# AtomGradient/swift-qwen3-tts

Measured on AMD Instinct MI355X. Metric: codec_tokens_per_s, higher is better.
Workload: dtype bf16

## Files before the change

### include/q3tts.h

```cpp
#ifndef Q3TTS_H
#define Q3TTS_H

#include <stddef.h>
#include <stdint.h>

#ifdef __cplusplus
extern "C" {
#endif

#define Q3TTS_ABI_VERSION 4

typedef struct q3tts_model q3tts_model;

typedef enum {
    Q3TTS_OK = 0,
    Q3TTS_ERR_MODEL_NOT_INITIALIZED = 1,
    Q3TTS_ERR_GENERATION_FAILED = 2,
    Q3TTS_ERR_INVALID_INPUT = 3,
    Q3TTS_ERR_AUDIO_DECODING_FAILED = 4,
    Q3TTS_ERR_AUDIO_ENCODING_FAILED = 5,
    Q3TTS_ERR_IO = 6,
    Q3TTS_ERR_DEVICE = 7,
    Q3TTS_ERR_CANCELLED = 8,
    Q3TTS_ERR_BUSY = 9
// ... 327 lines not shown
    float* rider_ss_out;
} q3tts_gemm_debug;
q3tts_status q3tts_debug_gemm(q3tts_model* m, q3tts_gemm_debug* a);

typedef struct {
    int32_t kind, geometry_only, split;
    int32_t B, Tmax, ppf, hist, margin;
    int32_t Cin, N, K, dil;
    int32_t ldx, ldo, ldr, ldx2;
    int32_t act, pre_act, shift, reflect, post_C;
    int32_t x_f32, res_is_out;
    int32_t family;
    int32_t BN;
    int32_t pro, pw_depth, KT, X32, CT2, PT, wdb;
    int32_t grid_x, grid_y, grid_z;
    int64_t lds_bytes;
    const int32_t* frames;
    const void* x;
    const float* x2;
    const float* w;
    const float* w2;
    const float* bias;
    const float* bias2;
    const float* scale;
    const float* snake_alpha;
    const float* snake_beta;
    const float* act2_alpha;
    const float* act2_beta;
    const float* post_alpha;
    const float* post_beta;
    const void* res;
    void* out;
    void* out2;
    float* pcm;
    int32_t* nonfinite;
} q3tts_conv_debug;
q3tts_status q3tts_debug_conv(q3tts_model* m, q3tts_conv_debug* a);

typedef struct {
    int32_t op, check_only;
    int32_t p[16];
    float f[4];
    const void* in[8];
    int64_t in_bytes[8];
    void* io[4];
    int64_t io_bytes[4];
} q3tts_rowop_debug;
q3tts_status q3tts_debug_rowop(q3tts_model* m, q3tts_rowop_debug* a);

typedef struct {
    float temperature;
    int32_t top_k;
    float top_p;
    float rep_penalty;
    uint64_t seed;
    uint32_t row0;
    int32_t mask_eos;
} q3tts_lm_sampling_params;
typedef struct {
    int32_t slot, n_trailing, max_frames;
    uint32_t row_key;
    int32_t text_open;
    int32_t pad_;
    q3tts_lm_sampling_params sp;
} q3tts_lm_admit_desc;
typedef struct {
    int32_t slot, src_row, n_new, close, max_frames, pad_;
} q3tts_lm_text_desc;
typedef struct {
    int32_t op, check_only;
    int32_t p[32];
    const void* in[14];
    int64_t in_bytes[14];
    void* io[18];
    int64_t io_bytes[18];
} q3tts_lmop_debug;
q3tts_status q3tts_debug_lmop(q3tts_model* m, q3tts_lmop_debug* a);

q3tts_status q3tts_debug_codec_stage(q3tts_model* m, const int32_t* codes, int32_t n_frames,
                                     const char* stage, float* out, int64_t cap_floats, int32_t* T, int32_t* C);

q3tts_status q3tts_debug_prefix_states(q3tts_model* m, int32_t* n_states, int64_t* device_bytes, int64_t* n_restored);

q3tts_status q3tts_debug_stretch_rows(q3tts_model* m, const float* x, const int32_t* lens, const int32_t* hops, int32_t B,
                                      int64_t x_stride, float* y, int64_t y_stride);

q3tts_status q3tts_debug_resample_ratio(q3tts_model* m, const float* x, const int32_t* lens, int32_t B, int64_t row_stride, int64_t in_units,
                                        int64_t out_units, int32_t centred, int32_t clamp, int32_t hist, float* y, int64_t y_stride);

q3tts_status q3tts_debug_codec_stream_slots(q3tts_model* m, const int32_t* codes, const int32_t* n_frames, int32_t n_reqs,
                                            int32_t max_frames, int32_t slots, int32_t burst, int32_t chunk_frames, int32_t window,
                                            int32_t lookahead, float* pcm);

q3tts_status q3tts_debug_build_decode_codes(q3tts_model* m, const int32_t* refs, const int32_t* ref_T, const int32_t* gen,
                                            const int32_t* n_frames, int32_t R, int32_t gen_stride, int32_t Fdec, int32_t misalign,
                                            int32_t* out);

void q3tts_debug_set_codec_scratch(uint64_t bytes);

void q3tts_debug_reload_env(void);

q3tts_status q3tts_debug_frontend_stage(q3tts_model* m, const float* audio, int64_t n_samples, const char* stage,
                                        float* out, int64_t cap_floats, int32_t* T, int32_t* C);

#ifdef __cplusplus
}
#endif
#endif
```

### swift-qwen3-tts_amd/csrc/api.cc

```cpp
#include <atomic>
#include <cmath>
#include <cstdio>
#include <cstring>
#include <thread>
#include <vector>

#include "codec.h"
#include "comm.h"
#include "engine.h"
#include "tokenizer.h"

using q3::EngineGroup;

struct q3tts_session {
    q3tts_model* m = nullptr;
};

struct q3tts_model {
    std::unique_ptr<EngineGroup> eng;
    std::unique_ptr<q3tts_session> session;
    std::atomic<std::thread::id> owner{std::thread::id()};
    std::atomic<int> depth{0};
};
struct q3tts_tokenizer {
// ... 556 lines not shown
    return guarded(m, [&] {
        Q3_CHECK(m && audio && out, 3, "Invalid input: null argument");
        Q3_CHECK(sample_rate == 24000, 3,
                 "Invalid input: Only 24kHz audio is supported for speaker embedding extraction");
        m->eng->lane0().speaker_embedding(audio, n_samples, out, cap);
        m->eng->timing = m->eng->lane0().timing;
    });
}

q3tts_status q3tts_debug_frontend_stage(q3tts_model* m, const float* audio, int64_t n_samples, const char* stage, float* out,
                                        int64_t cap_floats, int32_t* T, int32_t* C) {
    return guarded(m, [&] {
        Q3_CHECK(m && audio && stage && out && T && C, 3, "Invalid input: null argument");
        m->eng->lane0().debug_frontend_stage(audio, n_samples, stage, out, cap_floats, T, C);
    });
}

q3tts_status q3tts_tokenizer_load(const char* path, q3tts_tokenizer** out) {
    return guarded(nullptr, [&] {
        Q3_CHECK(path && out, 3, "Invalid input: null argument");
        auto t = std::make_unique<q3tts_tokenizer>();
        const std::string p = path;
        if (p.size() > 5 && p.compare(p.size() - 5, 5, ".json") == 0) t->tok.load_json_file(p);
        else t->tok.load(p);
        *out = t.release();
    });
}
void q3tts_tokenizer_free(q3tts_tokenizer* t) { delete t; }
q3tts_status q3tts_tokenizer_encode(const q3tts_tokenizer* t, const char* utf8, int32_t* ids, int32_t cap, int32_t* n) {
    return guarded(nullptr, [&] {
        Q3_CHECK(t && utf8 && n, 3, "Invalid input: null argument");
        const std::vector<int32_t> v = t->tok.encode(utf8);
        *n = int32_t(v.size());
        Q3_CHECK(ids == nullptr || cap >= *n, 3, "Invalid input: output buffer too small for the token ids");
        if (ids) std::memcpy(ids, v.data(), v.size() * 4);
    });
}

q3tts_status q3tts_last_timing(const q3tts_model* m, q3tts_timing* out) {
    if (!m || !out) return Q3TTS_ERR_INVALID_INPUT;
    *out = m->eng->timing;
    return Q3TTS_OK;
}

q3tts_status q3tts_debug_prepare_inputs(q3tts_model* m, const q3tts_request* req, uint16_t* input_embeds,
                                        int32_t cap_prompt, int32_t* n_prompt, uint16_t* trailing, int32_t cap_trailing,
                                        int32_t* n_trailing, uint16_t* tts_pad) {
    return guarded(m, [&] {
        Q3_CHECK(m && req && input_embeds && n_prompt && trailing && n_trailing && tts_pad, 3, "Invalid input: null argument");
        m->eng->lane0().debug_prepare_inputs(*req, input_embeds, cap_prompt, n_prompt, trailing, cap_trailing, n_trailing, tts_pad);
    });
}

q3tts_status q3tts_debug_generate_forced(q3tts_model* m, const q3tts_request* reqs, int32_t n_reqs,
                                         const q3tts_sampling* sampling, const int32_t* forced_codes, int32_t n_frames,
                                         uint16_t* talker_logits, uint16_t* cp_logits, int32_t* sampled) {
    return guarded(m, [&] {
        Q3_CHECK(m && reqs && n_frames > 0, 3, "Invalid input: null argument");
        q3tts_sampling sp;
        if (sampling) sp = *sampling;
        else q3tts_default_sampling(&sp);
        q3::DebugOpts d;
        d.forced_codes = forced_codes;
        d.frames = n_frames;
        d.talker_logits = talker_logits;
        d.cp_logits = cp_logits;
        d.sampled = sampled;
        std::vector<q3tts_result> res((size_t)(n_reqs));
        m->eng->generate(reqs, n_reqs, sp, nullptr, nullptr, res.data(), &d);
        q3tts_result_free(res.data(), n_reqs);
    });
}

q3tts_status q3tts_debug_sample(q3tts_model* m, const uint16_t* logits, int32_t rows, int32_t V,
                                const q3tts_sampling* sampling, const uint8_t* seen, int32_t suppress_lo,
                                int32_t suppress_hi, int32_t eos_id, uint32_t row0, uint32_t draw, int32_t* tokens) {
    return guarded(m, [&] {
        Q3_CHECK(m && logits && sampling && tokens, 3, "Invalid input: null argument");
        q3::check_row_sampling(*sampling, rows);
        m->eng->lane0().debug_sample(logits, rows, V, *sampling, seen, suppress_lo, suppress_hi, eos_id, row0, draw, tokens);
    });
}

q3tts_status q3tts_debug_text_resume(q3tts_model* m, int32_t H, int32_t V, const uint16_t* tables, const int32_t* codes,
                                     const uint16_t* text_row, uint16_t* out_h, float* out_ss, int32_t* out_state) {
    return guarded(m, [&] {
        Q3_CHECK(m, 3, "Invalid input: null argument");
        m->eng->lane0().debug_text_resume(H, V, tables, codes, text_row, out_h, out_ss, out_state);
    });
}

q3tts_status q3tts_debug_linear(q3tts_model* m, const uint16_t* x, const uint16_t* W, const uint16_t* bias, int32_t M,
                                int32_t K, int32_t N, uint16_t* y) {
    return guarded(m, [&] {
        Q3_CHECK(m && x && W && y, 3, "Invalid input: null argument");
        m->eng->lane0().debug_linear(x, W, bias, M, K, N, y);
    });
}

q3tts_status q3tts_debug_attention(q3tts_model* m, const q3tts_attn_debug* a) {
    return guarded(m, [&] {
        Q3_CHECK(m && a, 3, "Invalid input: null argument");
        m->eng->lane0().debug_attention(*a);
    });
}

q3tts_status q3tts_debug_gemm(q3tts_model* m, q3tts_gemm_debug* a) {
    if (a && a->geometry_only) {
        return guarded(nullptr, [&] {
            q3::GemmArgs ga{};
            q3::NormRowsArgs na{};
            q3::Engine::debug_gemm_check(*a, ga, na);
        });
    }
    return guarded(m, [&] {
        Q3_CHECK(m && a, 3, "Invalid input: null argument");
        m->eng->lane0().debug_gemm(*a);
    });
}

q3tts_status q3tts_debug_conv(q3tts_model* m, q3tts_conv_debug* a) {
    if (a && a->geometry_only) {
        return guarded(nullptr, [&] { q3::Engine::debug_conv_check(*a); });
    }
    return guarded(m, [&] {
        Q3_CHECK(m && a, 3, "Invalid input: null argument");
        m->eng->lane0().debug_conv(*a);
    });
}

q3tts_status q3tts_debug_rowop(q3tts_model* m, q3tts_rowop_debug* a) {
    if (a && a->check_only) {
        return guarded(nullptr, [&] { q3::Engine::debug_rowop_check(*a); });
    }
    return guarded(m, [&] {
        Q3_CHECK(m && a, 3, "Invalid input: null argument");
        m->eng->lane0().debug_rowop(*a);
    });
}

q3tts_status q3tts_debug_lmop(q3tts_model* m, q3tts_lmop_debug* a) {
    if (a && a->check_only) {
        return guarded(nullptr, [&] { q3::Engine::debug_lmop_check(*a); });
    }
    return guarded(m, [&] {
        Q3_CHECK(m && a, 3, "Invalid input: null argument");
        m->eng->lane0().debug_lmop(*a);
    });
}

q3tts_status q3tts_codec_decode_streamed(q3tts_model* m, const int32_t* codes, const int32_t* n_frames, int32_t batch, int32_t max_frames,
                                         int32_t chunk_frames, int32_t window, int32_t lookahead, float* pcm) {
    return guarded(m, [&] {
        Q3_CHECK(m && codes && n_frames && pcm, 3, "Invalid input: null argument");
        m->eng->lane0().codec_decode_streamed(codes, n_frames, batch, max_frames, chunk_frames, window, lookahead, pcm);
    });
}

q3tts_status q3tts_codec_decode_streamed_prefixed(q3tts_model* m, const int32_t* codes, const int32_t* n_prefix, const int32_t* n_frames,
                                                  int32_t batch, int32_t max_frames, int32_t chunk_frames, int32_t window, int32_t lookahead,
                                                  float* pcm) {
    return guarded(m, [&] {
        Q3_CHECK(m && codes && n_prefix && n_frames && pcm, 3, "Invalid input: null argument");
        m->eng->lane0().codec_decode_streamed_prefixed(codes, n_prefix, n_frames, batch, max_frames, chunk_frames, window, lookahead, pcm);
    });
}
// ... 55 lines not shown
```

### swift-qwen3-tts_amd/csrc/debug_env.cc

```cpp
#include <atomic>
#include <cstdlib>
#include <mutex>

#include "kernels.h"

namespace q3 {

namespace {
std::mutex g_mu;
std::atomic<const DebugEnv*> g_env{nullptr};

bool flag(const char* name) { return std::getenv(name) != nullptr; }
int number(const char* name, int dflt) {
    const char* e = std::getenv(name);
    return e && *e ? std::atoi(e) : dflt;
}

const DebugEnv* read_env() {
    DebugEnv* d = new DebugEnv{};
    d->gemm_no_row_split = flag("Q3TTS_GEMM_NO_ROW_SPLIT");
    d->gemm_one_pair = flag("Q3TTS_GEMM_ONE_PAIR");
    d->gemm_parent_forms = number("Q3TTS_GEMM_PARENT_FORMS", 0) != 0;
    d->no_tall_gemm = flag("Q3TTS_NO_TALL_GEMM");
    d->tall_shape = number("Q3TTS_TALL_SHAPE", 0);
    d->chunk_qsplit = number("Q3TTS_CHUNK_QSPLIT", 0);
    d->conv_no_pw = flag("Q3TTS_CONV_NO_PW");
    d->nt_off = std::getenv("Q3TTS_NT") && number("Q3TTS_NT", 1) == 0;
    d->serial_jobs = number("Q3TTS_SERIAL_JOBS", 0) != 0;
    d->fail_back_half = number("Q3TTS_TEST_FAIL_BACK_HALF", 0) != 0;
    d->no_prefix_cache = number("Q3TTS_NO_PREFIX_CACHE", 0) != 0;
    return d;
}
}

const DebugEnv& debug_env() {
    const DebugEnv* e = g_env.load(std::memory_order_acquire);
    if (!e) {
        std::lock_guard<std::mutex> lk(g_mu);
        e = g_env.load(std::memory_order_acquire);
        if (!e) {
            e = read_env();
            g_env.store(e, std::memory_order_release);
        }
    }
    return *e;
}

void debug_env_reload() {
    std::lock_guard<std::mutex> lk(g_mu);
    g_env.store(read_env(), std::memory_order_release);
}

}
```

### swift-qwen3-tts_amd/csrc/engine.cc

```cpp
#include "engine_stream.h"

#include "frontend.h"

namespace q3 {

namespace {
std::string lower(const std::string& s) {
    std::string o = s;
    for (auto& c : o) c = char(std::tolower((unsigned char)c));
    return o;
}
}

Engine::Engine(Model* model, const q3tts_load_opts& opts, float pitch) : m_(model), opts_(opts) {
    Q3_HIP(hipSetDevice(m_->device));
    {
        int least = 0, greatest = 0;
        Q3_HIP(hipDeviceGetStreamPriorityRange(&least, &greatest));
        Q3_HIP(hipStreamCreateWithPriority(&st_, hipStreamNonBlocking, greatest));
        Q3_HIP(hipStreamCreateWithPriority(&st_codec_, hipStreamNonBlocking, least));
        hipDeviceProp_t prop{};
        Q3_HIP(hipGetDeviceProperties(&prop, m_->device));
        int cus = prop.multiProcessorCount / 2;
        if (opts.codec_overlap_cus > 0) cus = opts.codec_overlap_cus;
// ... 59 lines not shown
    if (stager_.joinable()) {
        {
            std::lock_guard<std::mutex> lk(stage_mu_);
            stage_stop_ = true;
        }
        stage_cv_.notify_all();
        stager_.join();
    }
    for (auto& g : graphs_) (void)hipGraphExecDestroy(g.second);
    for (auto& g : qgraphs_) (void)hipGraphExecDestroy(g.second);
    for (auto& g : ographs_) (void)hipGraphExecDestroy(g.second);
    if (qws_) (void)hipFree(qws_);
    codec_.reset();
    fe_.reset();
    for (auto& L : fe_lanes_) {
        L.fe.reset();
        if (L.done) (void)hipEventDestroy(L.done);
        if (L.st) (void)hipStreamDestroy(L.st);
    }
    for (auto& J : jobs_) {
        for (auto& e : J.chunk_done)
            if (e) (void)hipEventDestroy(e);
        for (auto& e : J.ev_codec)
            if (e) (void)hipEventDestroy(e);
        if (J.ev_begin) (void)hipEventDestroy(J.ev_begin);
        if (J.ev_first_audio) (void)hipEventDestroy(J.ev_first_audio);
    }
    if (ws_) (void)hipFree(ws_);
    for (void* p : {(void*)forced_dev_, (void*)sampled_dev_, (void*)tl_dump_, (void*)cl_dump_})
        if (p) (void)hipFree(p);
    for (auto& e : ev_)
        if (e) (void)hipEventDestroy(e);
    for (auto& e : burst_ev_)
        if (e) (void)hipEventDestroy(e);
    for (auto& e : ev_fe_)
        if (e) (void)hipEventDestroy(e);
    if (fe_uploaded_) (void)hipEventDestroy(fe_uploaded_);
    if (stamps_) {
        unsigned long long h[64];
        if (hipMemcpy(h, stamps_, sizeof(h), hipMemcpyDeviceToHost) == hipSuccess && h[0] > 0) {
            static const char* nm[] = {"", "talker layers", "codec_head + norm + sampler (+ proj)", "predictor pair pass",
                                       "pass-0 head + sampler", "predictor passes 1..14 (layers)", "their heads + samplers", "frame_end"};
            std::fprintf(stderr, "[q3tts frame stamps] %llu frame steps\n", h[0]);
            for (int k = 1; k < 8; ++k) std::fprintf(stderr, "  %-40s %8.1f us per step\n", nm[k], double(h[k]) / 100.0 / double(h[0]));
        }
        (void)hipFree(stamps_);
    }
    if (st_codec_wide_) (void)hipStreamDestroy(st_codec_wide_);
    if (st_codec_part_) (void)hipStreamDestroy(st_codec_part_);
    if (st_codec_) (void)hipStreamDestroy(st_codec_);
    if (st_) (void)hipStreamDestroy(st_);
}

void Engine::build_cp_proj_tables() {
    if (cp_tables_ || !m_->has_cp_proj || std::getenv("Q3TTS_NO_PROJ_TABLES")) return;
    const TalkerConfig& t = m_->cfg.talker;
    const int H = t.hidden_size, CH = m_->cp.hidden, MBL = Mp_ / 16, Vc = t.cp.vocab_size, nss = CH / 16;
    const int ntab = t.num_code_groups - 2;
    if (ntab <= 0) return;
    std::lock_guard<std::mutex> lock(m_->lazy_mutex);
    if (m_->cp_pe.empty()) {
        for (int i = 0; i < ntab; ++i) {
            uint16_t* pe = nullptr;
            float* pss = nullptr;
            Q3_HIP(hipMalloc(reinterpret_cast<void**>(&pe), size_t(Vc) * CH * 2));
            m_->lazy_allocs.push_back(pe);
            Q3_HIP(hipMalloc(reinterpret_cast<void**>(&pss), size_t(Vc) * nss * 4));
            m_->lazy_allocs.push_back(pss);
            for (int c0 = 0; c0 < Vc; c0 += Mp_) {
                const int rows = std::min(Mp_, Vc - c0);
                launch_tile_rows(m_->cp_emb[size_t(i)] + size_t(c0) * H, H, cp_x_, MBL, rows, H, st_);
                GemmArgs p = gemm_args(m_->cp_proj, cp_x_, rows);
                p.epi = 3; p.y = cp_.h; p.yMB = MBL; p.resid = 0; p.ss_out = cp_.ss_a;
                launch_gemm_skinny(p, st_);
                launch_untile_rows(cp_.h, MBL, pe + size_t(c0) * CH, CH, rows, CH, st_);
                launch_ss_to_table(cp_.ss_a, Mp_, pss + size_t(c0) * nss, nss, rows, st_);
            }
            m_->cp_pe.push_back(pe);
            m_->cp_pss.push_back(pss);
        }
        Q3_HIP(hipStreamSynchronize(st_));
    }
    cp_tables_ = true;
}

void Engine::alloc_workspace() {
    const TalkerConfig& t = m_->cfg.talker;
    const int H = t.hidden_size, CH = t.cp.hidden_size, TH = t.text_hidden_size;
    const int qd = t.num_attention_heads * kHeadDim, kd = t.num_key_value_heads * kHeadDim;
    const int cqd = t.cp.num_attention_heads * kHeadDim, ckd = t.cp.num_key_value_heads * kHeadDim;
    const int L = t.num_hidden_layers, CL = t.cp.num_hidden_layers;
    kv_layer_stride_ = size_t(n_pages_) * t.num_key_value_heads * kPageTokens * kHeadDim;
    cp_kv_layer_stride_ = size_t(Bm_) * t.cp.num_key_value_heads * kPageTokens * kHeadDim;
    proj_cap_ = Bm_ * (2 * Pcap_ + 8);
    for (int pass = 0; pass < 2; ++pass) {
        Bump b{pass ? ws_ : nullptr};
        Bump& x = b;
        auto stream = [&](Stream& s, int hid, int q, int k, int inter_p, int vocab) {
            s.ld_qkv = q + 2 * k;
            s.ld_act = inter_p;
            s.ld_logits = vocab;
            s.h = x.take<uint16_t>(size_t(Mp_) * hid);
            s.xn = x.take<uint16_t>(size_t(Mp_) * hid);
            s.ss_a = x.take<float>(size_t(hid / 16) * Mp_);
            s.ss_b = x.take<float>(size_t(hid / 16) * Mp_);
            s.qkv = x.take<uint16_t>(size_t(Mp_) * s.ld_qkv);
            s.ao = x.take<uint16_t>(size_t(Mp_) * q);
            s.act = x.take<uint16_t>(size_t(Mp_) * inter_p);
            s.logits = b.take<uint16_t>(size_t(Mp_) * vocab);
        };
        stream(tk_, H, qd, kd, m_->talker.max_inter_p, t.vocab_size);
        stream(cp_, CH, cqd, ckd, m_->cp.max_inter_p, t.cp.vocab_size);
        cp_x_ = x.take<uint16_t>(size_t(Mp_) * H);
        cp_x2_ = x.take<uint16_t>(size_t(Mp_) * H);
        cp_ss2_ = x.take<float>(size_t(Mp_));
        kpool_ = b.take<uint16_t>(kv_layer_stride_ * L);
        vpool_ = b.take<uint16_t>(kv_layer_stride_ * L);
        cp_kpool_ = b.take<uint16_t>(cp_kv_layer_stride_ * CL);
        cp_vpool_ = b.take<uint16_t>(cp_kv_layer_stride_ * CL);
        block_table_ = b.take<int32_t>(size_t(Bm_) * max_pages_);
        cp_block_table_ = b.take<int32_t>(size_t(Bm_));
        kv_len_ = b.take<int32_t>(size_t(Bm_));
        cp_len_ = b.take<int32_t>(size_t(Bm_));
        n_frames_ = b.take<int32_t>(size_t(Bm_));
        max_frames_ = b.take<int32_t>(size_t(Bm_));
        trailing_idx_ = b.take<int32_t>(size_t(Bm_));
        n_trailing_ = b.take<int32_t>(size_t(Bm_));
        n_prompt_ = b.take<int32_t>(size_t(Bm_));
        cur_codes_ = b.take<int32_t>(size_t(Bm_) * 16);
        codes_ = b.take<int32_t>(size_t(Bm_) * Fcap_ * 16);
        active_ = b.take<uint8_t>(size_t(Bm_));
        finished_ = b.take<uint8_t>(size_t(Bm_));
        seen_ = b.take<uint8_t>(size_t(Bm_) * t.vocab_size);
        prompt_ = b.take<uint16_t>(size_t(Bm_) * Pcap_ * H);
        trailing_ = b.take<uint16_t>(size_t(Bm_) * Tcap_ * H);
        tts_pad_ = b.take<uint16_t>(size_t(H));
        sp_dev_ = b.take<SamplingParams>(size_t(Bm_));
        ids_dev_ = b.take<int32_t>(size_t(proj_cap_));
        proj_in_ = b.take<uint16_t>(size_t(64) * TH);
        proj_mid_ = b.take<uint16_t>(size_t(64) * TH);
        proj_out_ = b.take<uint16_t>(size_t(proj_cap_ + 64) * H);
        compose_a_ = b.take<int32_t>(size_t(3) * Bm_ * (Pcap_ + Tcap_));
        compose_b_ = nullptr;
        if (!pass) {
            ws_bytes_ = align_up(b.off, 256);
            Q3_HIP(hipMalloc(reinterpret_cast<void**>(&ws_), ws_bytes_));
            Q3_HIP(hipMemset(ws_, 0, ws_bytes_));
        }
    }
    std::vector<int32_t> cbt((size_t)(Bm_));
    for (int i = 0; i < Bm_; ++i) cbt[size_t(i)] = i;
    Q3_HIP(hipMemcpy(cp_block_table_, cbt.data(), cbt.size() * 4, hipMemcpyHostToDevice));
}

GemmArgs Engine::gemm_args(const LinearW& L, const uint16_t* x, int M) const {
    GemmArgs a{};
    a.W = L.w;
    a.Wsb = L.sb;
    a.x = x;
    a.xMB = Mp_ / 16;
    a.M = M;
    a.Mpad = int(align_up(size_t(M), 16));
    a.N = L.Np;
    a.K = L.Kp;
    a.bias = L.bias;
    a.ss_ld = Mp_;
    return a;
}

void Engine::enqueue_layers(const StackW& s, Stream& w, int B, uint16_t* kpool, uint16_t* vpool, size_t layer_stride,
                            const int32_t* block_table, int max_pages, const int32_t* kv_len, const uint8_t* active,
                            int ss_count_in, int fixed_len, int chunk, const int32_t* chunk_n_prompt, int chunk_r_base) {
    const int H = s.hidden, MBL = Mp_ / 16, tiles = H / 16;
    const int M = B * (chunk > 1 ? chunk : 1);
    Q3_CHECK(M <= Mp_, 7, "internal error: chunk does not fit the activation buffers");
    const bool row_norm = M > 64;
    const bool prologue_qkv = H <= 2048 && !row_norm, prologue_mlp = H <= 2048 && !row_norm;
    const bool nt_off = debug_env().nt_off;
    const bool is_talker = &s == &m_->talker;
    const int ntw = is_talker && !nt_off ? 1 : 0;
    const int ntkv = ntw;
    auto norm_into_xn = [&](const uint16_t* nw, const float* ss, int ss_count) {
        NormRowsArgs n{};
        n.h = w.h; n.hMB = MBL; n.w = nw; n.eps = s.eps; n.out = w.xn; n.outMB = MBL; n.M = M; n.H = H;
        if (row_norm && H <= 2048) { n.ss_in = ss; n.ss_count = ss_count; n.ss_ld = Mp_; }
        launch_norm_rows(n, counted());
    };
    for (size_t l = 0; l < s.layers.size(); ++l) {
        const LayerW& L = s.layers[l];
        if (!prologue_qkv) norm_into_xn(L.ln1, w.ss_a, (l == 0) ? ss_count_in : tiles);
        GemmArgs q = gemm_args(L.qkv, prologue_qkv ? w.h : w.xn, M);
        q.epi = 0; q.y = w.qkv; q.ldy = w.ld_qkv; q.nt_weights = ntw;
        if (prologue_qkv) {
            q.norm_w = L.ln1; q.ss_in = w.ss_a; q.ss_count = (l == 0) ? ss_count_in : tiles; q.norm_dim = H; q.norm_eps = s.eps;
        }
        AttnArgs at{};
        at.qkv = w.qkv; at.ld = w.ld_qkv; at.qn_w = L.qn; at.kn_w = L.kn; at.eps = s.eps;
        at.rope_cos = s.rope_cos; at.rope_sin = s.rope_sin;
        at.kpool = kpool + l * layer_stride; at.vpool = vpool + l * layer_stride;
        at.block_table = block_table; at.max_pages = max_pages; at.kv_len = kv_len; at.active = active;
        at.out = w.ao; at.outMB = MBL; at.n_heads = s.n_heads; at.n_kv = s.n_kv; at.B = B;
        at.fixed_len = fixed_len; at.identity_pages = fixed_len >= 0 ? 1 : 0;
        at.chunk = chunk; at.chunk_n_prompt = chunk_n_prompt; at.chunk_r_base = chunk_r_base;
        at.scale = powf(float(kHeadDim), -0.5f);
        at.nt_kv = ntkv;
        launch_gemm_skinny(q, counted());
        launch_attn_decode(at, counted());
        GemmArgs o = gemm_args(L.o, w.ao, M);
        o.epi = 3; o.y = w.h; o.yMB = MBL; o.resid = 1; o.ss_out = w.ss_b; o.nt_weights = ntw;
        launch_gemm_skinny(o, counted());
        if (!prologue_mlp) norm_into_xn(L.ln2, w.ss_b, tiles);
        GemmArgs g = gemm_args(L.gateup, prologue_mlp ? w.h : w.xn, M);
        g.epi = 2; g.y = w.act; g.yMB = MBL; g.nt_weights = ntw;
        if (prologue_mlp) {
            g.norm_w = L.ln2; g.ss_in = w.ss_b; g.ss_count = tiles; g.norm_dim = H; g.norm_eps = s.eps;
        }
        launch_gemm_skinny(g, counted());
        GemmArgs d = gemm_args(L.down, w.act, M);
        d.epi = 3; d.y = w.h; d.yMB = MBL; d.resid = 1; d.ss_out = w.ss_a; d.nt_weights = ntw;
        launch_gemm_skinny(d, counted());
    }
}

void Engine::enqueue_talker_step(int B, bool with_head) {
    (void)with_head;
    enqueue_layers(m_->talker, tk_, B, kpool_, vpool_, kv_layer_stride_, block_table_, max_pages_, kv_len_, active_, 1, -1, 1, nullptr, 0);
}

void Engine::enqueue_cp_pass(int B, bool from_talker, int head, int cp_pos, bool projected) {
    const TalkerConfig& t = m_->cfg.talker;
    const int H = t.hidden_size, CH = m_->cp.hidden, MBL = Mp_ / 16;
    int ss_count = 1;
    auto talker_norm_into = [&](uint16_t* dst, float* ss_out) {
        NormRowsArgs n{};
        n.h = tk_.h; n.hMB = MBL; n.w = m_->talker.final_norm; n.eps = m_->talker.eps;
        n.out = dst; n.outMB = MBL; n.ss_out = ss_out; n.M = B; n.H = H;
        launch_norm_rows(n, counted());
    };
    if (m_->has_cp_proj && projected) {
        ss_count = CH / 16;
    } else if (m_->has_cp_proj) {
        if (from_talker) talker_norm_into(cp_x2_, nullptr);
        GemmArgs p = gemm_args(m_->cp_proj, from_talker ? cp_x2_ : cp_x_, B);
        p.epi = 3; p.y = cp_.h; p.yMB = MBL; p.resid = 0; p.ss_out = cp_.ss_a;
        launch_gemm_skinny(p, counted());
        ss_count = CH / 16;
    } else if (from_talker) {
        talker_norm_into(cp_.h, cp_.ss_a);
    }
    enqueue_layers(m_->cp, cp_, B, cp_kpool_, cp_vpool_, cp_kv_layer_stride_, cp_block_table_, 1, cp_len_, nullptr, ss_count, cp_pos, 1, nullptr, 0);
}

FrameEndArgs Engine::frame_end_args(int B) const {
    const TalkerConfig& t = m_->cfg.talker;
    FrameEndArgs fe{};
    fe.cur_codes = cur_codes_; fe.codec_emb = m_->codec_emb; fe.cp_emb = m_->cp_emb_dev;
    fe.trailing = trailing_; fe.n_trailing = n_trailing_; fe.trailing_idx = trailing_idx_; fe.Tmax = Tcap_;
    fe.tts_pad = tts_pad_; fe.h = tk_.h; fe.hMB = Mp_ / 16; fe.ss_out = tk_.ss_a; fe.H = t.hidden_size; fe.B = B; fe.groups = t.num_code_groups;
    fe.n_frames = n_frames_; fe.max_frames = max_frames_; fe.finished = finished_; fe.active = active_; fe.cp_len = cp_len_;
    fe.text_open = frame_text_open_; fe.starved = frame_text_open_ ? starved_ : nullptr;
    return fe;
}

void Engine::enqueue_frame(int B, const DebugOpts* dbg) {
    struct Count {
        Engine* e;
        int B;
        ~Count() { e->frame_launches_[B] = e->launches_; }
    } count{this, B};
    launches_ = 0;
    const TalkerConfig& t = m_->cfg.talker;
    const int H = t.hidden_size, V = t.vocab_size, Vc = t.cp.vocab_size, CH = t.cp.hidden_size;
    const int groups = t.num_code_groups, MBL = Mp_ / 16;
    stamp(0);
    enqueue_talker_step(B, true);
    stamp(1);
    uint16_t* next_x = m_->has_cp_proj ? cp_x_ : cp_.h;
    float* next_ss = m_->has_cp_proj ? nullptr : cp_.ss_a;
    const bool pair = 2 * B <= Mp_;
    {
        GemmArgs hd = gemm_args(m_->codec_head, tk_.h, B);
        hd.epi = 0; hd.y = tk_.logits; hd.ldy = tk_.ld_logits;
        hd.norm_w = m_->talker.final_norm; hd.ss_in = tk_.ss_a; hd.ss_count = H / 16; hd.norm_dim = H; hd.norm_eps = m_->talker.eps;
        bool rode = false;
        if (pair) {
            NormRowsArgs n{};
            n.h = tk_.h; n.hMB = MBL; n.w = m_->talker.final_norm; n.eps = m_->talker.eps;
            n.out = next_x; n.outMB = MBL; n.ss_out = next_ss; n.M = B; n.H = H;
            rode = launch_gemm_skinny_with_norm_rows(hd, n, st_);
            if (rode) ++launches_;
            else launch_norm_rows(n, counted());
        }
        if (!rode) launch_gemm_skinny(hd, counted());
    }
    SamplerArgs sa{};
    sa.logits = tk_.logits; sa.ldl = tk_.ld_logits; sa.V = V; sa.sp = sp_dev_; sa.is_talker = 1;
    sa.suppress_lo = V - 1024; sa.suppress_hi = V; sa.eos_id = t.codec_eos_token_id;
    sa.seen = seen_; sa.cb = 0; sa.n_frames = n_frames_; sa.max_frames = max_frames_;
    sa.finished = finished_; sa.active = active_; sa.kv_len = kv_len_; sa.advance = 1; sa.advance_gate = active_;
    sa.cur_codes = cur_codes_; sa.codes = codes_; sa.Fmax = Fcap_;
    sa.forced = dbg ? forced_dev_ : nullptr; sa.forced_frames = dbg ? dbg->frames : 0;
    sa.sampled = dbg ? sampled_dev_ : nullptr;
    sa.emb = m_->codec_emb; sa.emb_ld = H; sa.next_MB = MBL; sa.H = H; sa.B = B;
    if (pair) {
        sa.next_x = next_x; sa.next_row0 = B; sa.next_ss = next_ss ? next_ss + B : nullptr;
    } else {
        sa.next_x = m_->has_cp_proj ? cp_x_ : cp_x2_; sa.next_ss = m_->has_cp_proj ? nullptr : cp_ss2_;
    }
    sa.logits_dump = (dbg && dbg->talker_logits) ? tl_dump_ : nullptr; sa.dump_ld = V; sa.dump_off = 0;
    sa.row_key = frame_row_key_;
    if (pair) {
        launch_sampler(sa, counted());
        int ss_count = 1;
        if (m_->has_cp_proj) {
            GemmArgs p = gemm_args(m_->cp_proj, cp_x_, 2 * B);
            p.epi = 3; p.y = cp_.h; p.yMB = MBL; p.resid = 0; p.ss_out = cp_.ss_a;
            launch_gemm_skinny(p, counted());
            ss_count = CH / 16;
        }
        stamp(2);
        enqueue_layers(m_->cp, cp_, B, cp_kpool_, cp_vpool_, cp_kv_layer_stride_, cp_block_table_, 1, cp_len_, nullptr, ss_count, 0, 2,
                       nullptr, 0);
        stamp(3);
    } else {
        launch_sampler(sa, counted());
        enqueue_cp_pass(B, true, -1, 0);
        if (!m_->has_cp_proj) {
            launch_copy_rows(cp_x2_, 0, cp_.h, 0, 1, Mp_ * H, counted());
            launch_copy_rows(reinterpret_cast<const uint16_t*>(cp_ss2_), 0, reinterpret_cast<uint16_t*>(cp_.ss_a), 0, 1, Mp_ * 2, counted());
        }
    }
    const FrameEndArgs fe = frame_end_args(B);
    bool fe_done = false;
    for (int i = 0; i < groups - 1; ++i) {
        const bool second_of_pair = pair && i == 0;
        const int Mh = second_of_pair ? 2 * B : B;
        if (!second_of_pair) {
            enqueue_cp_pass(B, false, i, i + 1, cp_tables_ && i >= 1);
            stamp(5);
        }
        {
            GemmArgs lh = gemm_args(m_->lm_head[size_t(i)], cp_.h, Mh);
            lh.epi = 0; lh.y = cp_.logits; lh.ldy = cp_.ld_logits;
            lh.norm_w = m_->cp.final_norm; lh.ss_in = cp_.ss_a; lh.ss_count = CH / 16; lh.norm_dim = CH; lh.norm_eps = m_->cp.eps;
            launch_gemm_skinny(lh, counted());
        }
        SamplerArgs sc{};
        sc.logits = cp_.logits + (second_of_pair ? size_t(B) * cp_.ld_logits : 0); sc.ldl = cp_.ld_logits; sc.V = Vc; sc.sp = sp_dev_;
        sc.is_talker = 0;
        sc.eos_id = -1; sc.cb = i + 1; sc.n_frames = n_frames_; sc.max_frames = max_frames_;
        sc.finished = finished_; sc.active = active_; sc.kv_len = cp_len_; sc.advance = 1; sc.advance_gate = nullptr;
        sc.cur_codes = cur_codes_; sc.codes = codes_; sc.Fmax = Fcap_;
        sc.forced = dbg ? forced_dev_ : nullptr; sc.forced_frames = dbg ? dbg->frames : 0;
        sc.sampled = dbg ? sampled_dev_ : nullptr;
        if (i + 1 < groups - 1) {
            sc.emb = m_->cp_emb[size_t(i)]; sc.emb_ld = H; sc.next_x = next_x; sc.next_MB = MBL; sc.next_ss = next_ss;
        }
        sc.H = H; sc.B = B;
        if (cp_tables_ && i + 1 < groups - 1) {
            sc.emb = m_->cp_pe[size_t(i)]; sc.emb_ld = CH; sc.H = CH; sc.next_x = cp_.h;
            sc.emb_ss = m_->cp_pss[size_t(i)]; sc.nss = CH / 16; sc.next_ss = cp_.ss_a; sc.next_ss_ld = Mp_;
        }
        sc.logits_dump = (dbg && dbg->cp_logits) ? cl_dump_ : nullptr; sc.dump_ld = (groups - 1) * Vc; sc.dump_off = i * Vc;
        sc.row_key = frame_row_key_;
        if (i == groups - 2 && Vc <= 2048) {
            launch_sampler_with_frame_end(sc, fe, counted());
            fe_done = true;
        } else {
            launch_sampler(sc, counted());
        }
        stamp(second_of_pair ? 4 : 6);
    }
    if (!fe_done) launch_frame_end(fe, counted());
    stamp(7);
}

hipGraphExec_t Engine::frame_graph(int B) {
    std::map<int, hipGraphExec_t>& graphs = frame_text_open_ ? ographs_ : frame_row_key_ ? qgraphs_ : graphs_;
    auto it = graphs.find(B);
    if (it != graphs.end()) return it->second;
    hipGraph_t g = nullptr;
    Q3_HIP(hipStreamBeginCapture(st_, hipStreamCaptureModeThreadLocal));
    try {
        enqueue_frame(B, nullptr);
    } catch (...) {
        (void)hipStreamEndCapture(st_, &g);
        if (g) (void)hipGraphDestroy(g);
        throw;
    }
    Q3_HIP(hipStreamEndCapture(st_, &g));
    hipGraphExec_t ge = nullptr;
    Q3_HIP(hipGraphInstantiate(&ge, g, nullptr, nullptr, 0));
    Q3_HIP(hipGraphDestroy(g));
    graphs[B] = ge;
    return ge;
}

void Engine::check_reference(const float* ref_audio, int64_t n_ref_samples, const int32_t* ref_text_ids, int n_ref_text_ids) const {
    Q3_CHECK(m_->has_codec, 1, "Model not initialized: Speech tokenizer not loaded");
    Q3_CHECK(m_->has_codec_encoder, 1,
             "Model not initialized: Voice cloning (ICL mode) requires the speech tokenizer encoder. Make sure to load a model "
             "with encoder weights.");
    Q3_CHECK(ref_audio && n_ref_samples > 0, 3, "Invalid input: reference audio is empty");
    {
        bool finite = true;
        for (int64_t i = 0; i < n_ref_samples; ++i) finite = finite && (std::fabs(ref_audio[i]) <= 3.0e38f);
        Q3_CHECK(finite, 3, "Invalid input: reference audio holds non-finite samples");
    }
    Q3_CHECK(ref_text_ids && n_ref_text_ids >= 5, 3, "Invalid input: ref_text_ids must hold the chat-template tokens");
}

ResolvedRequest Engine::resolve(const q3tts_request& r, const q3tts_sampling& sp, const Voice* voice) const {
    const ModelConfig& cfg = m_->cfg;
    const TalkerConfig& t = cfg.talker;
    ResolvedRequest o;
    if (r.speed != 0.0f) {
        Q3_CHECK(codec_ && codec_->request_speeds(), 3,
                 "Invalid input: q3tts_request.speed needs a handle loaded with q3tts_load_opts.request_speeds");
        const int hs = codec_->speed_plan().hs_of(r.speed);
        Q3_CHECK(hs != 0, 3, "Invalid input: q3tts_request.speed must be 0 (the handle's speed) or between 0.5 and 2.0");
        if (hs != codec_->stretch_hs()) {
            Q3_CHECK(sp.audio_chunk_frames == 0 || (sp.audio_window_frames > 0 && codec_->stream_own_hops()), 3,
                     "Invalid input: a request speed other than the handle's with audio_chunk_frames > 0 needs audio_window_frames > 0 "
                     "(streamed audio) and a handle without output_sample_rate");
            o.hs = hs;
        }
    }
    Q3_CHECK(r.text_ids && r.n_text_ids >= 4, 3, "Invalid input: text_ids must hold the chat-template tokens");
    Q3_CHECK(r.route >= 0 && r.route <= 2, 3, "Invalid input: unknown q3tts_request.route");
    o.text_ids.assign(r.text_ids, r.text_ids + r.n_text_ids);
    const bool have_instruct = r.instruct_ids && r.n_instruct_ids > 0;
    const std::string type = cfg.tts_model_type;
    auto speaker_list = [&]() {
        std::string s;
        for (size_t i = 0; i < speakers.size(); ++i) s += (i ? ", " : "") + speakers[i];
        return s;
    };
    bool use_speaker = false, use_instruct = false;
    if (r.ref_audio != nullptr || voice) {
        if (!voice) check_reference(r.ref_audio, r.n_ref_samples, r.ref_text_ids, r.n_ref_text_ids);
        Q3_CHECK(r.n_text_ids >= 8, 3, "Invalid input: text_ids must hold the chat-template tokens");
        Q3_CHECK(m_->codec_enc.bins <= t.vocab_size && m_->codec_enc.bins <= t.cp.vocab_size, 3,
                 "Invalid input: encoder codebook larger than the codec embedding tables");
        o.clone = true;
// ... 745 lines not shown
    });
}

int Engine::open_job(const q3tts_request* reqs, int n, const q3tts_sampling& sp, const DebugOpts* dbg, std::vector<ResolvedRequest>& rr,
                     double& t_start, const Voice* const* voices) {
    Q3_CHECK(n >= 1 && n <= Bm_, 3, "Invalid input: batch size must be between 1 and max_batch");
    Q3_CHECK(m_->cfg.talker.num_code_groups == 16, 3, "Invalid input: num_code_groups must be 16");
    Q3_CHECK(sp.audio_chunk_frames >= 0, 3, "Invalid input: audio_chunk_frames must not be negative");
    if (sp.audio_chunk_frames > 0 && sp.audio_window_frames > 0 && m_->has_codec)
        Q3_CHECK(sp.audio_chunk_frames >= codec_->hist_frames(), 3,
                 "Invalid input: audio_chunk_frames of a streamed decode must be at least " + std::to_string(codec_->hist_frames()));
    int slot = -1;
    for (int i = 0; i < kJobSlots; ++i)
        if (!jobs_[i].busy && slot < 0) slot = i;
    Q3_CHECK(slot >= 0, 3, "Invalid input: two jobs are already outstanding (q3tts_generate_end must be called first)");
    t_start = now_s();
    Q3_HIP(hipEventRecord(jobs_[slot].ev_begin, st_));
    for (int i = 0; i < n; ++i) rr.push_back(resolve(reqs[i], sp, voices ? voices[i] : nullptr));
    if (dbg)
        for (auto& r : rr) r.max_frames = dbg->frames;
    for (auto& r : rr) Q3_CHECK(r.max_frames <= Fcap_, 3, "Invalid input: max_tokens exceeds the configured max_frames");
    if (m_->has_codec == false)
        throw Error(1, "Model not initialized: Speech tokenizer not loaded");
    return slot;
}

int Engine::reserve_rows(const std::vector<ResolvedRequest>& rr, const std::vector<int>& np, const std::vector<int>& nt,
                         const q3tts_sampling& sp) {
    const int n = int(rr.size());
    int Pmax = 0;
    for (int p : np) Pmax = std::max(Pmax, p);
    std::vector<int32_t> bt((size_t)(n) * max_pages_, 0), maxf((size_t)(n)), ntr((size_t)(n)), npr((size_t)(n));
    int next_page = 0;
    for (int b = 0; b < n; ++b) {
        const int need = ceil_div(np[size_t(b)] + rr[size_t(b)].max_frames + 1, kPageTokens);
        Q3_CHECK(need <= max_pages_ && next_page + need <= n_pages_, 3, "Invalid input: KV pool exhausted");
        for (int i = 0; i < need; ++i) bt[size_t(b) * max_pages_ + i] = next_page++;
        maxf[size_t(b)] = rr[size_t(b)].max_frames;
        ntr[size_t(b)] = nt[size_t(b)];
        npr[size_t(b)] = np[size_t(b)];
    }
    Q3_CHECK(Pmax + *std::max_element(maxf.begin(), maxf.end()) + 1 <= m_->talker.max_pos, 3,
             "Invalid input: sequence longer than the RoPE table");
    Q3_HIP(hipMemcpyAsync(block_table_, bt.data(), bt.size() * 4, hipMemcpyHostToDevice, st_));
    Q3_HIP(hipMemcpyAsync(max_frames_, maxf.data(), size_t(n) * 4, hipMemcpyHostToDevice, st_));
    Q3_HIP(hipMemcpyAsync(n_trailing_, ntr.data(), size_t(n) * 4, hipMemcpyHostToDevice, st_));
    Q3_HIP(hipMemcpyAsync(n_prompt_, npr.data(), size_t(n) * 4, hipMemcpyHostToDevice, st_));
    for (int32_t* p : {kv_len_, cp_len_, n_frames_, trailing_idx_}) Q3_HIP(hipMemsetAsync(p, 0, size_t(n) * 4, st_));
    Q3_HIP(hipMemsetAsync(active_, 0, size_t(n), st_));
    Q3_HIP(hipMemsetAsync(finished_, 0, size_t(n), st_));
    Q3_HIP(hipMemsetAsync(seen_, 0, size_t(n) * m_->cfg.talker.vocab_size, st_));
    Q3_HIP(hipMemsetAsync(codes_, 0, size_t(n) * Fcap_ * 16 * 4, st_));
    upload_sampling(sp, row_offset + sp.row_base, n);
    return Pmax;
}

void Engine::debug_buffers(int n, const DebugOpts& dbg) {
    const TalkerConfig& t = m_->cfg.talker;
    const int V = t.vocab_size, Vc = t.cp.vocab_size;
    for (void* p : {(void*)forced_dev_, (void*)sampled_dev_, (void*)tl_dump_, (void*)cl_dump_})
        if (p) (void)hipFree(p);
    forced_dev_ = sampled_dev_ = nullptr;
    tl_dump_ = cl_dump_ = nullptr;
    const size_t nf = size_t(n) * dbg.frames;
    if (dbg.forced_codes) {
        for (size_t i = 0; i < nf * 16; ++i) {
            const int32_t c = dbg.forced_codes[i];
            Q3_CHECK(c >= 0 && c < ((i & 15) == 0 ? V : Vc), 3, "Invalid input: forced code outside its vocabulary");
        }
        Q3_HIP(hipMalloc(reinterpret_cast<void**>(&forced_dev_), nf * 16 * 4));
        Q3_HIP(hipMemcpy(forced_dev_, dbg.forced_codes, nf * 16 * 4, hipMemcpyHostToDevice));
    }
    Q3_HIP(hipMalloc(reinterpret_cast<void**>(&sampled_dev_), nf * 16 * 4));
    Q3_HIP(hipMemset(sampled_dev_, 0xff, nf * 16 * 4));
    if (dbg.talker_logits) Q3_HIP(hipMalloc(reinterpret_cast<void**>(&tl_dump_), nf * V * 2));
    if (dbg.cp_logits) Q3_HIP(hipMalloc(reinterpret_cast<void**>(&cl_dump_), nf * (t.num_code_groups - 1) * Vc * 2));
}

int Engine::frame_loop(Job& J, const std::vector<ResolvedRequest>& rr, const q3tts_sampling& sp, q3tts_event_cb cb, void* user,
                       const DebugOpts* dbg, StreamedDecode& sd) {
    const int n = J.n;
    const bool use_graph = opts_.use_graph && !dbg;
    build_cp_proj_tables();
    hipGraphExec_t ge = use_graph ? frame_graph(n) : nullptr;
    int frames_cap = 0;
    for (auto& r : rr) frames_cap = std::max(frames_cap, r.max_frames);
    std::vector<int32_t> h_nframes((size_t)(n), 0);
    std::vector<uint8_t> h_fin((size_t)(n), 0);
    std::vector<int> reported((size_t)(n), 0);
    int launched = 0;
    const bool fixed_len = sp.force_frames > 0 || dbg;
    const int burst_frames = std::max(1, max_inflight_frames / job_chains / 2);
    hipEvent_t ring[2] = {burst_ev_[0], burst_ev_[1]};
    int bursts = 0;
    bool done = false;
    while (!done && launched < frames_cap) {
        if (bursts >= 2) Q3_HIP(hipEventSynchronize(ring[bursts & 1]));
        int burst = std::min(burst_frames, frames_cap - launched);
        if (sd.on) {
            const int need = std::min(frames_cap, sd.next_need(launched, sp.audio_chunk_frames, std::max(0, sp.audio_lookahead_frames)));
            if (need > launched) burst = std::min(burst, need - launched);
        }
        for (int i = 0; i < burst; ++i) {
            if (use_graph) Q3_HIP(hipGraphLaunch(ge, st_));
            else enqueue_frame(n, dbg);
        }
        launched += burst;
        if (!(fixed_len && !cb)) {
            Q3_HIP(hipMemcpyAsync(h_nframes.data(), n_frames_, size_t(n) * 4, hipMemcpyDeviceToHost, st_));
            Q3_HIP(hipMemcpyAsync(h_fin.data(), finished_, size_t(n), hipMemcpyDeviceToHost, st_));
        }
        Q3_HIP(hipEventRecord(ring[bursts & 1], st_));
        ++bursts;
        if (fixed_len && !cb) {
            if (sd.on) {
                for (int b = 0; b < n; ++b) sd.avail[size_t(b)] = std::min(launched, rr[size_t(b)].max_frames);
                sd.feed(launched);
            }
            continue;
        }
        Q3_HIP(hipEventSynchronize(ring[(bursts - 1) & 1]));
        done = true;
        for (int b = 0; b < n; ++b) done = done && h_fin[size_t(b)];
        if (sd.on) {
            for (int b = 0; b < n; ++b) {
                sd.avail[size_t(b)] = h_nframes[size_t(b)];
                sd.fin[size_t(b)] = h_fin[size_t(b)];
            }
            sd.feed(launched);
            fire_chunks(J, J.n_chunks, &sd.avail, false);
        }
        if (cb)
            for (int b = 0; b < n; ++b) emit_tokens(cb, user, b, request_base + b, h_nframes[size_t(b)], reported[size_t(b)]);
    }
    Q3_HIP(hipEventRecord(ev_[2], st_));
    Q3_HIP(hipMemcpyAsync(h_nframes.data(), n_frames_, size_t(n) * 4, hipMemcpyDeviceToHost, st_));
    Q3_HIP(hipStreamSynchronize(st_));
    if (dbg) {
        const TalkerConfig& t = m_->cfg.talker;
        const size_t nf = size_t(n) * dbg->frames;
        if (dbg->sampled) Q3_HIP(hipMemcpy(dbg->sampled, sampled_dev_, nf * 16 * 4, hipMemcpyDeviceToHost));
        if (dbg->talker_logits) Q3_HIP(hipMemcpy(dbg->talker_logits, tl_dump_, nf * t.vocab_size * 2, hipMemcpyDeviceToHost));
        if (dbg->cp_logits)
            Q3_HIP(hipMemcpy(dbg->cp_logits, cl_dump_, nf * (t.num_code_groups - 1) * t.cp.vocab_size * 2, hipMemcpyDeviceToHost));
    }
    J.frames.assign(h_nframes.begin(), h_nframes.end());
    return launched;
}

void Engine::hand_off(Job& J, const std::vector<ResolvedRequest>& rr, StreamedDecode& sd, int launched, bool overlapped) {
    const int n = J.n;
    bool any_clone = false;
    std::vector<int> dframes((size_t)(n), 0);
    int Fdec = 0;
    for (int b = 0; b < n; ++b) {
        const int F = J.frames[size_t(b)];
        any_clone = any_clone || rr[size_t(b)].clone;
        J.ref_T[size_t(b)] = rr[size_t(b)].clone ? rr[size_t(b)].ref_T : 0;
        J.target_tokens[size_t(b)] = rr[size_t(b)].target_token_count;
        dframes[size_t(b)] = F > 0 ? F + J.ref_T[size_t(b)] : 0;
        Fdec = std::max(Fdec, dframes[size_t(b)]);
    }
    J.Fdec = sd.on ? (sd.ss ? sd.stride : Fcap_) : Fdec;
    J.codes_host.resize(size_t(n) * Fcap_ * 16);
    Q3_HIP(hipMemcpyAsync(J.codes_host.data(), codes_, J.codes_host.size() * 4, hipMemcpyDeviceToHost, st_));
    if (sd.on) {
// ... 485 lines not shown
```

### swift-qwen3-tts_amd/csrc/engine.h

```cpp
#pragma once
#include <atomic>
#include <cstdlib>
#include <functional>
#include <map>
#include <memory>
#include <condition_variable>
#include <mutex>
#include <thread>
#include <string>
#include <unordered_map>
#include <vector>

#include "../../include/q3tts.h"
#include "kernels.h"
#include "model.h"
#include "pitch_plan.h"
#include "queue_slots.h"
#include "resample_plan.h"
#include "session_queue.h"
#include "stretch_plan.h"

namespace q3 {

struct DebugOpts {
// ... 84 lines not shown
        entries.push_back(std::move(n));
    }
    void drop(const Voice* v) {
        std::lock_guard<std::mutex> lk(mu);
        for (size_t i = entries.size(); i-- > 0;)
            if (entries[i]->voice == v) entries.erase(entries.begin() + ptrdiff_t(i));
    }
    void stats(int32_t* n_entries, int64_t* bytes, int64_t* n_restored) {
        std::lock_guard<std::mutex> lk(mu);
        *n_entries = int32_t(entries.size());
        *bytes = 0;
        for (auto& e : entries) *bytes += int64_t(e->bytes);
        *n_restored = restored.load();
    }
};

struct QueueItem {
    int ticket = -1;
    ResolvedRequest rr;
    SamplingParams params{};
};

struct RequestSource {
    virtual ~RequestSource() = default;
    virtual bool take(QueueItem& out) = 0;
    virtual q3tts_result* result(int ticket) = 0;
    virtual void complete(int) {}
    virtual bool open_ended() const { return false; }
    virtual bool wait_for_work() { return false; }
    virtual bool has_cancels() { return false; }
    virtual void take_cancels(std::vector<int>& out) { out.clear(); }
    virtual void complete_cancelled(int) {}
    virtual void progress(int , int ) {}
    struct TextAppend {
        int ticket = -1;
        std::vector<int32_t> ids;
        bool final = false;
    };
    virtual bool open_text() const { return false; }
    virtual bool has_appends() { return false; }
    virtual void take_appends(std::vector<TextAppend>& out) { out.clear(); }
    virtual void wait_for_text(bool ) {}
    virtual void text_progress(int , int ) {}
};

struct QueueShared {
    RequestSource* src = nullptr;
    uint32_t row_base = 0;
    int voice_ref_max = -1;
    bool stream_reference = false;
    int ref_max = 0;
    PrefixCache* prefix_cache = nullptr;
};

class Engine {
  public:
    Engine(Model* model, const q3tts_load_opts& opts, float pitch = 0.0f);
    ~Engine();

    Model& model() { return *m_; }
    const q3tts_load_opts& opts() const { return opts_; }
    std::string last_error;
    q3tts_timing timing{};

    void generate(const q3tts_request* reqs, int n, const q3tts_sampling& sp, q3tts_event_cb cb, void* user,
                  q3tts_result* results, const DebugOpts* dbg, const Voice* const* voices = nullptr);
    static constexpr int kJobSlots = 2;
    int begin(const q3tts_request* reqs, int n, const q3tts_sampling& sp, q3tts_event_cb cb, void* user, const DebugOpts* dbg,
              bool overlapped,
              bool background = false, const Voice* const* voices = nullptr);
    void end(int job, q3tts_result* results);
    bool job_outstanding() const;
    int text_cap() const { return Tcap_; }
    void prepare_job_pair();
    void drain();
    ResolvedRequest check_queued(const q3tts_request& r, const q3tts_sampling& sp, const Voice* voice = nullptr,
                                 bool open_text = false) const;
    void check_stream_chunk(int chunk_frames) const;
    void run_queued(QueueShared& q, int slots, const q3tts_sampling& sp, q3tts_event_cb cb, void* user);
    void debug_prepare_inputs(const q3tts_request& req, uint16_t* input_embeds, int cap_prompt, int* n_prompt,
                              uint16_t* trailing, int cap_trailing, int* n_trailing, uint16_t* tts_pad);
    void debug_sample(const uint16_t* logits, int rows, int V, const q3tts_sampling& sp, const uint8_t* seen,
                      int suppress_lo, int suppress_hi, int eos_id, uint32_t row0, uint32_t draw, int32_t* tokens);
    void debug_text_resume(int H, int V, const uint16_t* tables, const int32_t* codes, const uint16_t* text, uint16_t* out_h,
                           float* out_ss, int32_t* out_state);
    void debug_linear(const uint16_t* x, const uint16_t* W, const uint16_t* bias, int M, int K, int N, uint16_t* y);
    void debug_attention(const q3tts_attn_debug& a);
    static void debug_gemm_check(q3tts_gemm_debug& d, GemmArgs& ga, NormRowsArgs& na);
    void debug_gemm(q3tts_gemm_debug& d);
    static void debug_conv_check(q3tts_conv_debug& d);
    void debug_conv(q3tts_conv_debug& d);
    static void debug_rowop_check(const q3tts_rowop_debug& d);
    void debug_rowop(q3tts_rowop_debug& d);
    static void debug_lmop_check(const q3tts_lmop_debug& d);
    void debug_lmop(q3tts_lmop_debug& d);
    void debug_build_decode_codes(const int32_t* refs, const int32_t* ref_T, const int32_t* gen, const int32_t* n_frames, int R,
                                  int gen_stride, int Fdec, bool misalign, int32_t* out);
    void codec_decode(const int32_t* codes, const int32_t* n_frames, int batch, int max_frames, float* pcm,
                      int64_t* audio_lengths);
    void codec_decode_streamed(const int32_t* codes, const int32_t* n_frames, int batch, int max_frames, int chunk_frames, int window,
                               int lookahead, float* pcm);
    void codec_decode_streamed_prefixed(const int32_t* codes, const int32_t* n_prefix, const int32_t* n_frames, int batch, int max_frames,
                                        int chunk_frames, int window, int lookahead, float* pcm);
    void debug_codec_stream_slots(const int32_t* codes, const int32_t* n_frames, int n_reqs, int max_frames, int slots, int burst,
                                  int chunk_frames, int window, int lookahead, float* pcm);
    void debug_codec_stage(const int32_t* codes, int n_frames, const char* stage, float* out, int64_t cap, int* T, int* C);
    int codec_encode(const float* audio, int64_t n_samples, int32_t* codes, int cap_frames);
    int encoded_frames(int64_t n_samples) const;
    void speaker_embedding(const float* audio, int64_t n_samples, float* out, int cap);
    std::unique_ptr<Voice> create_voice(const float* audio, int64_t n_samples, const int32_t* ref_text_ids, int n_ref_text_ids,
                                        int sample_rate = 24000);
    void resample(const float* in, int64_t n_in, int in_rate, int out_rate, bool centred, float* out, int64_t cap, int64_t* n_out);
    void time_stretch(const float* in, int64_t n_in, float speed, bool causal, float* out, int64_t cap, int64_t* n_out);
    void debug_stretch_rows(const float* x, const int32_t* lens, const int32_t* hops, int B, int64_t x_stride, float* y, int64_t y_stride);
    void pitch_shift(const float* in, int64_t n_in, float semitones, float* out, int64_t cap, int64_t* n_out);
    void debug_resample_ratio(const float* x, const int32_t* lens, int B, int64_t row_stride, int64_t in_units, int64_t out_units, bool centred,
                              bool clamp, int hist, float* y, int64_t y_stride);
    void debug_frontend_stage(const float* audio, int64_t n_samples, const char* stage, float* out, int64_t cap, int* T, int* C);

    std::vector<std::string> speakers;
    const CodecRunner* codec_runner() const { return codec_.get(); }

  private:
    Model* m_;
  public:
    uint32_t row_offset = 0;
    std::mutex* cb_mutex = nullptr;
    int request_base = 0;
    int max_inflight_frames = 16;
    int job_chains = 1;
  private:
    q3tts_load_opts opts_;
    hipStream_t st_ = nullptr;
    hipStream_t st_codec_ = nullptr;
    hipStream_t st_codec_part_ = nullptr;
    hipStream_t st_codec_wide_ = nullptr;
    hipStream_t masked_stream(int cus, int total);
    hipStream_t codec_stream(bool overlapped, bool wide = false);
    hipEvent_t ev_[4] = {nullptr, nullptr, nullptr, nullptr};
    hipEvent_t burst_ev_[2] = {nullptr, nullptr};
    hipEvent_t ev_fe_[2] = {nullptr, nullptr};
    hipEvent_t fe_uploaded_ = nullptr;
    int Bm_ = 0, Mp_ = 0;
    int Pcap_ = 0, Tcap_ = 0, Fcap_ = 0, max_pages_ = 0, n_pages_ = 0;

    uint8_t* ws_ = nullptr;
    size_t ws_bytes_ = 0;
    struct Stream {
        uint16_t *h, *xn, *qkv, *ao, *act, *logits;
        float *ss_a, *ss_b;
        int ld_qkv, ld_act, ld_logits;
    } tk_{}, cp_{};
    uint16_t* cp_x_ = nullptr;
    uint16_t* cp_x2_ = nullptr;
    bool cp_tables_ = false;
    void build_cp_proj_tables();
    float* cp_ss2_ = nullptr;
    uint16_t *kpool_ = nullptr, *vpool_ = nullptr, *cp_kpool_ = nullptr, *cp_vpool_ = nullptr;
    size_t kv_layer_stride_ = 0, cp_kv_layer_stride_ = 0;
    int32_t *block_table_ = nullptr, *cp_block_table_ = nullptr;
    int32_t *kv_len_ = nullptr, *cp_len_ = nullptr, *n_frames_ = nullptr, *max_frames_ = nullptr;
    int32_t *trailing_idx_ = nullptr, *n_trailing_ = nullptr, *n_prompt_ = nullptr, *cur_codes_ = nullptr, *codes_ = nullptr;
    uint8_t *active_ = nullptr, *finished_ = nullptr, *seen_ = nullptr;
    uint16_t *prompt_ = nullptr, *trailing_ = nullptr, *tts_pad_ = nullptr;
    SamplingParams* sp_dev_ = nullptr;
    int32_t* ids_dev_ = nullptr;
    uint16_t *proj_in_ = nullptr, *proj_mid_ = nullptr, *proj_out_ = nullptr;
    int proj_cap_ = 0;
    int32_t *compose_a_ = nullptr, *compose_b_ = nullptr;
    int32_t *forced_dev_ = nullptr, *sampled_dev_ = nullptr;
    uint16_t *tl_dump_ = nullptr, *cl_dump_ = nullptr;

    struct Job {
        std::atomic<bool> busy{false};
        uint64_t seq = 0;
        std::vector<ResolvedRequest> rr;
        std::vector<int> np;
        q3tts_sampling sp{};
        bool overlapped = false;
        bool frontend = false;
        bool background = false;
        int back = 0;
        int back_status = 0;
        std::string back_err;
        int n = 0, Fdec = 0, up = 0;
        std::vector<int> row_hs;
        std::vector<int> row_up;
        std::vector<int> frames, ref_T, target_tokens, n_prompt;
        std::vector<int> req_index;
        std::vector<q3tts_result*> row_out;
        std::vector<double> row_span;
        std::vector<std::vector<int32_t>> ref_code0;
        std::vector<int32_t> codes_host;
        DevBuf<int32_t> dec_codes;
        std::vector<const Voice*> voices;
        DevBuf<int32_t> gen_codes;
        std::vector<DecodeRowDesc> row_desc;
        DevBuf<DecodeRowDesc> row_desc_dev;
        PinnedBuf<float> pcm_host;
        hipEvent_t ev_codec[2] = {nullptr, nullptr};
        PinnedBuf<int32_t> nf_host;
        PinnedBuf<int32_t> nf_chunk_host;
        std::vector<int> held_from;
        hipEvent_t ev_begin = nullptr, ev_first_audio = nullptr;
        std::vector<hipEvent_t> chunk_done;
        int n_chunks = 0, chunk_frames = 0;
        bool streamed = false;
        bool prefixed = false;
        int chunks_fired = 0;
        double t_first_audio = 0;
        q3tts_timing timing{};
        double t_start = 0, t_done = 0;
        q3tts_event_cb cb = nullptr;
        void* user = nullptr;
        int request_base = 0;
        bool decoded = false;
        std::vector<int64_t> row_cut, row_ns;
        std::vector<MallocPtr<float>> st_pcm;
        std::vector<MallocPtr<int32_t>> st_codes;
        int stage = 0;
        std::string stage_err;
        void reset(int rows, int upsample);
        void clear_chunk_flags(int frames);
    } jobs_[kJobSlots];
    void start_decode(Job& J, const std::vector<int>& dframes, bool overlapped, const int32_t* codes_host);
    void publish_job(Job& J, q3tts_event_cb cb, void* user, int request_base, double t_start, bool stage);
    void release_job(Job& J);
    void compute_cuts(Job& J);
    void fire_chunks(Job& J, int upto, const std::vector<int>* known, bool wait);
    std::unique_lock<std::mutex> cb_lock();
    void emit_tokens(q3tts_event_cb cb, void* user, int row, int request, int nf, int& reported);
    void stage_rows(Job& J);
    std::vector<int> redo_rows_fp32(Job& J);
    struct ExactDecode {
        PinnedBuf<float> pcm;
        PinnedBuf<int32_t> nf;
        int Fd = 0, up = 0;
    };
    ExactDecode decode_rows_fp32(const std::vector<int>& dframes, const std::function<void(int, int32_t*, hipStream_t)>& place,
// ... 4 lines not shown
    std::thread stager_;
    std::mutex stage_mu_;
    std::condition_variable stage_cv_;
    bool stage_stop_ = false;
    uint64_t job_seq_ = 0;

    unsigned long long* stamps_ = nullptr;
    void stamp(int k) {
        if (stamps_) launch_stamp(stamps_, stamps_ + 63, k, counted());
    }
    hipStream_t counted() {
        ++launches_;
        return st_;
    }
    int launches_ = 0;
    std::map<int, int> frame_launches_;
    std::map<int, hipGraphExec_t> graphs_;
    std::unique_ptr<CodecRunner> codec_;
    std::unique_ptr<VoiceFrontEnd> fe_;
    DevBuf<float> ref_audio_dev_;
    DevBuf<int32_t> ref_codes_dev_;
    DevBuf<uint16_t> extra_;
    DevBuf<float> spk_f32_;
    struct FeLane {
        hipStream_t st = nullptr;
        hipEvent_t done = nullptr;
        std::unique_ptr<VoiceFrontEnd> fe;
        DevBuf<float> spk;
    };
    std::vector<FeLane> fe_lanes_;
    const float* upload_audio(const float* audio, int64_t n);
    struct ResamplerDev {
        ResamplePlan plan;
        DevBuf<float> tab;
    };
    std::vector<std::unique_ptr<ResamplerDev>> resamplers_;
    DevBuf<float> rs_out_dev_;
    DevBuf<int32_t> rs_len_dev_;
    struct StretchDev {
        StretchPlan plan;
        DevBuf<float> fade;
    };
    std::vector<std::unique_ptr<StretchDev>> stretchers_;
    DevBuf<float> dbg_fade_all_;
    const ResamplerDev& resampler(int in_rate, int out_rate);
    std::vector<std::unique_ptr<ResamplerDev>> ratios_;
    const ResamplerDev& ratio_resampler(int64_t in_units, int64_t out_units);
    DevBuf<float> ps_mid_dev_;
    const float* resample_upload(const float* audio, int64_t n, int in_rate, int out_rate, bool centred, int64_t* n_out);
    bool prepare_clone_rows(std::vector<ResolvedRequest>& reqs);

    void alloc_workspace();
    ResolvedRequest resolve(const q3tts_request& r, const q3tts_sampling& sp, const Voice* voice = nullptr) const;
    void check_reference(const float* ref_audio, int64_t n_ref_samples, const int32_t* ref_text_ids, int n_ref_text_ids) const;
    int open_job(const q3tts_request* reqs, int n, const q3tts_sampling& sp, const DebugOpts* dbg, std::vector<ResolvedRequest>& rr,
                 double& t_start, const Voice* const* voices);
    int reserve_rows(const std::vector<ResolvedRequest>& rr, const std::vector<int>& np, const std::vector<int>& nt,
                     const q3tts_sampling& sp);
    void debug_buffers(int n, const DebugOpts& dbg);
    struct StreamedDecode;
    struct SlotStream;
    int frame_loop(Job& J, const std::vector<ResolvedRequest>& rr, const q3tts_sampling& sp, q3tts_event_cb cb, void* user,
                   const DebugOpts* dbg, StreamedDecode& sd);
    void hand_off(Job& J, const std::vector<ResolvedRequest>& rr, StreamedDecode& sd, int launched, bool overlapped);
    void back_half(Job& J, const std::vector<ResolvedRequest>& rr, const std::vector<int>& np, const q3tts_sampling& sp,
                   q3tts_event_cb cb, void* user, const DebugOpts* dbg, bool streamed, bool overlapped, double t_start);
    void worker_loop();
    std::thread worker_;
    std::mutex work_mu_;
    std::condition_variable work_cv_;
    Job* work_ = nullptr;
    bool work_stop_ = false;
    void job_timing(Job& J, const std::vector<int>& np, int launched);
    void upload_sampling(const q3tts_sampling& sp, uint32_t row0, int n);
    int64_t kv_bytes(int n_prompt, int frames) const;
    int launches_per_step(int B) const;
    void assemble_prompts(const std::vector<ResolvedRequest>& reqs, std::vector<int>& n_prompt, std::vector<int>& n_trailing,
                          const std::vector<int>* trailing_rows = nullptr);
    void enqueue_prefill(Stream& w, int n, int Pmax, const int32_t* block_table, int32_t* kv_len, const int32_t* n_prompt,
                         uint8_t* active);
    void project_rows(const std::vector<int32_t>& ids, int rows);
    void enqueue_layers(const StackW& s, Stream& w, int B, uint16_t* kpool, uint16_t* vpool, size_t layer_stride,
                        const int32_t* block_table, int max_pages, const int32_t* kv_len, const uint8_t* active,
                        int ss_count_in, int fixed_len, int chunk, const int32_t* chunk_n_prompt, int chunk_r_base);
    void enqueue_talker_step(int B, bool with_head);
    void enqueue_cp_pass(int B, bool from_talker, int head, int cp_pos, bool projected = false);
    void enqueue_frame(int B, const DebugOpts* dbg);
    FrameEndArgs frame_end_args(int B) const;
    hipGraphExec_t frame_graph(int B);
    const uint32_t* frame_row_key_ = nullptr;
    std::map<int, hipGraphExec_t> qgraphs_;
    uint8_t* qws_ = nullptr;
    Stream qk_{};
    int32_t *q_bt_ = nullptr, *q_kv_len_ = nullptr, *q_n_prompt_ = nullptr;
    uint8_t* q_active_ = nullptr;
    AdmitDesc* q_desc_ = nullptr;
    std::vector<AdmitDesc> q_desc_host_;
    uint32_t* row_key_ = nullptr;
    uint8_t *text_open_ = nullptr, *starved_ = nullptr;
    const uint8_t* frame_text_open_ = nullptr;
    std::map<int, hipGraphExec_t> ographs_;
    TextAppendDesc* q_text_desc_ = nullptr;
    std::vector<TextAppendDesc> q_text_desc_host_;
    std::vector<int32_t> q_text_ids_;
    std::vector<int32_t> q_host_;
    void ensure_queue_ws();
    struct QueueRun;
    struct QLive;
    void apply_text_appends(QueueShared& q, std::vector<QSlot>& sl, std::unordered_map<int, QLive>& live);
    int admit(QueueShared& q, std::vector<QSlot>& sl, std::unordered_map<int, QLive>& live);
    void cancel_slots(uint64_t mask, int slots);
    GemmArgs gemm_args(const LinearW& L, const uint16_t* x, int M) const;
};


class Session;

class EngineGroup {
  public:
    EngineGroup(std::unique_ptr<Model> model, const q3tts_load_opts& opts, float pitch = 0.0f);
    Model& model() { return *model_; }
    ~EngineGroup();
    Engine& lane0() {
        lanes_[0]->drain();
        return *lanes_[0];
    }
    int n_lanes() const { return int(lanes_.size()); }
    const CodecRunner* codec_runner() const { return lanes_[0]->codec_runner(); }
    const q3tts_load_opts& opts() const { return opts_; }
    void generate(const q3tts_request* reqs, int n, const q3tts_sampling& sp, q3tts_event_cb cb, void* user,
                  q3tts_result* results, const DebugOpts* dbg, const Voice* const* voices = nullptr);
    Voice* create_voice(const float* audio, int64_t n_samples, const int32_t* ref_text_ids, int n_ref_text_ids, int sample_rate = 24000);
    void free_voice(Voice* v);
    bool mine(const Voice* v) const;
    PrefixCache& prefix_cache() { return prefix_cache_; }
    int begin(const q3tts_request* reqs, int n, const q3tts_sampling& sp, q3tts_event_cb cb, void* user, bool more_follows);
    void end(int job, q3tts_result* results);
    void generate_queued(const q3tts_request* reqs, int n, int slots, const q3tts_sampling& sp, q3tts_event_cb cb, void* user,
                         q3tts_result* results, const Voice* const* voices = nullptr);
    Session* open_session(const q3tts_session_opts& so, const q3tts_sampling& sp, q3tts_event_cb cb, void* user);
    Session* session() const { return session_.get(); }
    int close_session(bool drain);
    std::string last_error;
    q3tts_timing timing{};
    std::vector<std::string> speakers;

  private:
    std::unique_ptr<Session> session_;
    void check_queue_open(int slots, const q3tts_sampling& sp) const;
    template <class F>
    static void run_lanes(int L, bool serial, F&& fn);
    struct Parked {
        bool busy = false;
        std::vector<q3tts_result> results;
        q3tts_timing timing{};
    } parked_[Engine::kJobSlots];
    std::unique_ptr<Model> model_;
    q3tts_load_opts opts_;
    std::mutex cb_mutex_;
    std::vector<std::unique_ptr<Engine>> lanes_;
    std::vector<std::unique_ptr<Voice>> voices_;
    PrefixCache prefix_cache_;
    void check_voices(const q3tts_request* reqs, int n, const Voice* const* voices) const;
    std::unique_ptr<Engine> ctx1_;
    int last_ctx_ = 1;
    bool background_ = false;
    Engine* free_context();
};

// ... 50 lines not shown
```

### swift-qwen3-tts_amd/csrc/engine_debug.cc

```cpp
#include "engine_stream.h"

#include "frontend.h"

namespace q3 {

void Engine::debug_frontend_stage(const float* audio, int64_t n_samples, const char* stage, float* out, int64_t cap, int* T, int* C) {
    Q3_CHECK(fe_ != nullptr, 1, "Model not initialized: Speech tokenizer encoder not available");
    Q3_CHECK(audio && n_samples > 0 && stage, 3, "Invalid input: empty audio or stage name");
    const float* a = upload_audio(audio, n_samples);
    StageCapture cap_s;
    cap_s.name = stage;
    static const char* kSpeaker[] = {"mel", "h0", "h1", "h2", "h3", "mfa", "pooled"};
    bool is_spk = false;
    for (const char* s : kSpeaker) is_spk = is_spk || cap_s.name == s;
    if (is_spk) {
        Q3_CHECK(m_->has_speaker_encoder, 1, "Model not initialized: Speaker encoder not available for this model");
        spk_f32_.grow(size_t(m_->cfg.talker.hidden_size));
        fe_->speaker_embedding(a, n_samples, spk_f32_, &cap_s);
    } else {
        Q3_CHECK(m_->has_codec_encoder, 1, "Model not initialized: Speech tokenizer encoder not available");
        const int Tq = fe_->encoded_frames(n_samples);
        ref_codes_dev_.grow(size_t(16) * Tq);
        fe_->encode(a, n_samples, ref_codes_dev_, &cap_s);
    }
    Q3_HIP(hipStreamSynchronize(st_));
    Q3_CHECK(!cap_s.data.empty(), 3, std::string("Invalid input: unknown front-end stage '") + stage + "'");
    Q3_CHECK(int64_t(cap_s.data.size()) <= cap, 3, "Invalid input: output buffer too small");
    std::memcpy(out, cap_s.data.data(), cap_s.data.size() * 4);
    *T = cap_s.T;
    *C = cap_s.C;
}

void Engine::debug_prepare_inputs(const q3tts_request& req, uint16_t* input_embeds, int cap_prompt, int* n_prompt,
                                  uint16_t* trailing, int cap_trailing, int* n_trailing, uint16_t* tts_pad) {
    q3tts_sampling sp{};
    q3tts_default_sampling(&sp);
    std::vector<ResolvedRequest> rr{resolve(req, sp)};
    if (rr[0].clone) prepare_clone_rows(rr);
    std::vector<int> np, nt;
    assemble_prompts(rr, np, nt);
    const int H = m_->cfg.talker.hidden_size;
    Q3_CHECK(np[0] <= cap_prompt && nt[0] <= cap_trailing, 3, "Invalid input: output buffers too small");
    Q3_HIP(hipStreamSynchronize(st_));
    Q3_HIP(hipMemcpy(input_embeds, prompt_, size_t(np[0]) * H * 2, hipMemcpyDeviceToHost));
    Q3_HIP(hipMemcpy(trailing, trailing_, size_t(nt[0]) * H * 2, hipMemcpyDeviceToHost));
    Q3_HIP(hipMemcpy(tts_pad, tts_pad_, size_t(H) * 2, hipMemcpyDeviceToHost));
    *n_prompt = np[0];
    *n_trailing = nt[0];
}

void Engine::debug_sample(const uint16_t* logits, int rows, int V, const q3tts_sampling& sp, const uint8_t* seen,
                          int suppress_lo, int suppress_hi, int eos_id, uint32_t row0, uint32_t draw, int32_t* tokens) {
    Q3_CHECK(rows >= 1 && rows <= Bm_ && V <= m_->cfg.talker.vocab_size, 3, "debug_sample: rows/V out of range");
    Q3_CHECK(draw % 16 == 0, 3, "debug_sample: draw must be a multiple of 16 (frame * 16)");
    const int Vt = m_->cfg.talker.vocab_size;
    Q3_HIP(hipMemcpy2D(tk_.logits, size_t(Vt) * 2, logits, size_t(V) * 2, size_t(V) * 2, size_t(rows), hipMemcpyHostToDevice));
    if (seen) Q3_HIP(hipMemcpy(seen_, seen, size_t(rows) * V, hipMemcpyHostToDevice));
    std::vector<int32_t> fr((size_t)(rows), int32_t(draw / 16)), big((size_t)(rows), 1 << 30);
    Q3_HIP(hipMemcpy(n_frames_, fr.data(), size_t(rows) * 4, hipMemcpyHostToDevice));
    Q3_HIP(hipMemcpy(max_frames_, big.data(), size_t(rows) * 4, hipMemcpyHostToDevice));
    Q3_HIP(hipMemset(finished_, 0, size_t(rows)));
    Q3_HIP(hipMemset(active_, 1, size_t(rows)));
    std::vector<SamplingParams> sph;
    for (int r = 0; r < rows; ++r) sph.push_back(fold_sampling(sp, r, row0));
    Q3_HIP(hipMemcpy(sp_dev_, sph.data(), sph.size() * sizeof(SamplingParams), hipMemcpyHostToDevice));
    SamplerArgs sa{};
    sa.logits = tk_.logits; sa.ldl = Vt; sa.V = V; sa.sp = sp_dev_;
    sa.is_talker = (eos_id >= 0 || suppress_hi > suppress_lo || seen) ? 1 : 0;
    sa.suppress_lo = suppress_lo; sa.suppress_hi = suppress_hi; sa.eos_id = eos_id;
    sa.seen = seen ? seen_ : nullptr; sa.cb = 0; sa.n_frames = n_frames_; sa.max_frames = max_frames_;
    sa.finished = finished_; sa.active = active_; sa.kv_len = kv_len_; sa.advance = 0;
    sa.cur_codes = cur_codes_; sa.codes = codes_; sa.Fmax = 0; sa.B = rows; sa.H = m_->cfg.talker.hidden_size;
    launch_sampler(sa, st_);
    Q3_HIP(hipStreamSynchronize(st_));
    std::vector<int32_t> cc((size_t)(rows) * 16);
    Q3_HIP(hipMemcpy(cc.data(), cur_codes_, cc.size() * 4, hipMemcpyDeviceToHost));
    for (int r = 0; r < rows; ++r) tokens[r] = cc[size_t(r) * 16];
    Q3_HIP(hipMemset(seen_, 0, size_t(rows) * V));
}

void Engine::debug_linear(const uint16_t* x, const uint16_t* W, const uint16_t* bias, int M, int K, int N, uint16_t* y) {
    Q3_CHECK(M >= 1 && M <= 1024 && K % 8 == 0 && N >= 1, 3, "debug_linear: unsupported shape");
    const int Kp = int(align_up(size_t(K), 128)), Np = int(align_up(size_t(N), 16)), Mp = int(align_up(size_t(M), 16));
    uint16_t *dW = nullptr, *dWt = nullptr, *dx = nullptr, *dy = nullptr, *db = nullptr;
    Q3_HIP(hipMalloc(reinterpret_cast<void**>(&dW), size_t(N) * K * 2));
    Q3_HIP(hipMalloc(reinterpret_cast<void**>(&dWt), size_t(Np) * Kp * 2));
    Q3_HIP(hipMalloc(reinterpret_cast<void**>(&dx), size_t(Mp) * Kp * 2));
    Q3_HIP(hipMalloc(reinterpret_cast<void**>(&dy), size_t(Mp) * Np * 2));
    Q3_HIP(hipMalloc(reinterpret_cast<void**>(&db), size_t(Np) * 2));
    Q3_HIP(hipMemset(dWt, 0, size_t(Np) * Kp * 2));
    Q3_HIP(hipMemset(dx, 0, size_t(Mp) * Kp * 2));
    Q3_HIP(hipMemset(db, 0, size_t(Np) * 2));
    Q3_HIP(hipMemcpy(dW, W, size_t(N) * K * 2, hipMemcpyHostToDevice));
    uint16_t* dxl = nullptr;
    Q3_HIP(hipMalloc(reinterpret_cast<void**>(&dxl), size_t(Mp) * Kp * 2));
    Q3_HIP(hipMemset(dxl, 0, size_t(Mp) * Kp * 2));
    Q3_HIP(hipMemcpy2D(dxl, size_t(Kp) * 2, x, size_t(K) * 2, size_t(K) * 2, size_t(M), hipMemcpyHostToDevice));
    launch_tile_rows(dxl, Kp, dx, Mp / 16, Mp, Kp, st_);
    if (bias) Q3_HIP(hipMemcpy(db, bias, size_t(N) * 2, hipMemcpyHostToDevice));
    launch_tile_weights(dW, N, K, dWt, Kp / 128, 0, 1, st_);
    LinearW L;
    L.w = dWt; L.bias = bias ? db : nullptr; L.N = N; L.K = K; L.Np = Np; L.Kp = Kp;
    GemmArgs ga{};
    ga.W = dWt; ga.x = dx; ga.xMB = Mp / 16; ga.M = M; ga.Mpad = Mp; ga.N = Np; ga.K = Kp; ga.epi = 0; ga.y = dy; ga.ldy = Np;
    ga.bias = L.bias; ga.ss_ld = Mp;
    launch_gemm_skinny(ga, st_);
    Q3_HIP(hipStreamSynchronize(st_));
    Q3_HIP(hipMemcpy2D(y, size_t(N) * 2, dy, size_t(Np) * 2, size_t(N) * 2, size_t(M), hipMemcpyDeviceToHost));
    for (void* p : {(void*)dW, (void*)dWt, (void*)dx, (void*)dxl, (void*)dy, (void*)db})
        if (p) (void)hipFree(p);
}

void Engine::debug_text_resume(int H, int V, const uint16_t* tables, const int32_t* codes, const uint16_t* text, uint16_t* out_h,
                               float* out_ss, int32_t* out_state) {
    Q3_CHECK(H >= 128 && H <= 4096 && H % 128 == 0 && V >= 1 && V <= 4096, 3, "debug_text_resume: H must be a multiple of 128 up to 4096, V up to 4096");
    Q3_CHECK(tables && codes && text && out_h && out_ss && out_state, 3, "Invalid input: null argument");
    for (int g = 0; g < 16; ++g) Q3_CHECK(codes[g] >= 0 && codes[g] < V, 3, "debug_text_resume: code outside the tables");
    constexpr int B = 2, row = 1, Tmax = 2;
    DevBuf<uint16_t> d_tab, d_trailing, d_pad, d_h, d_hl, d_text;
    DevBuf<const uint16_t*> d_cp;
    DevBuf<int32_t> d_i32;
    DevBuf<uint8_t> d_u8;
    DevBuf<float> d_ss;
    DevBuf<TextAppendDesc> d_desc;
    d_tab.grow(size_t(16) * V * H);
    d_trailing.grow(size_t(B) * Tmax * H);
    d_pad.grow(size_t(H));
    d_h.grow(size_t(16) * H);
    d_hl.grow(size_t(16) * H);
    d_text.grow(size_t(H));
    d_cp.grow(15);
    d_i32.grow(32 + 10);
    d_u8.grow(8);
    d_ss.grow(B);
    d_desc.grow(1);
    Q3_HIP(hipMemcpy(d_tab, tables, size_t(16) * V * H * 2, hipMemcpyHostToDevice));
    Q3_HIP(hipMemcpy(d_text, text, size_t(H) * 2, hipMemcpyHostToDevice));
    Q3_HIP(hipMemset(d_pad, 0, size_t(H) * 2));
    std::vector<const uint16_t*> cp(15);
    for (int g = 1; g < 16; ++g) cp[size_t(g - 1)] = d_tab + size_t(g) * V * H;
    Q3_HIP(hipMemcpy(d_cp, cp.data(), 15 * sizeof(const uint16_t*), hipMemcpyHostToDevice));
    int32_t* cur = d_i32;
    int32_t *n_tr = cur + 32, *t_idx = n_tr + 2, *n_fr = t_idx + 2, *max_fr = n_fr + 2, *cp_len = max_fr + 2;
    uint8_t *fin = d_u8, *act = fin + 2, *topen = act + 2, *starved = topen + 2;
    FrameEndArgs fe{};
    fe.cur_codes = cur; fe.codec_emb = d_tab; fe.cp_emb = d_cp;
    fe.trailing = d_trailing; fe.n_trailing = n_tr; fe.trailing_idx = t_idx; fe.Tmax = Tmax;
    fe.tts_pad = d_pad; fe.h = d_h; fe.hMB = 1; fe.ss_out = d_ss; fe.H = H; fe.B = B; fe.groups = 16;
    fe.n_frames = n_fr; fe.max_frames = max_fr; fe.finished = fin; fe.active = act; fe.cp_len = cp_len;
    fe.text_open = topen; fe.starved = starved;
    auto reset = [&](int n_trailing, int open) {
        std::vector<int32_t> hi(42, 0);
        for (int g = 0; g < 16; ++g) hi[size_t(16 + g)] = codes[g];
        hi[32 + row] = n_trailing;
        hi[38] = hi[39] = 100;
        hi[40] = hi[41] = 15;
        const uint8_t hu[8] = {1, 0, 0, 1, 0, uint8_t(open), 0, 0};
        const float hs[2] = {-1.f, -1.f};
        Q3_HIP(hipMemcpy(d_i32, hi.data(), hi.size() * 4, hipMemcpyHostToDevice));
        Q3_HIP(hipMemcpy(d_u8, hu, 8, hipMemcpyHostToDevice));
        Q3_HIP(hipMemcpy(d_ss, hs, 8, hipMemcpyHostToDevice));
// ... 540 lines not shown
```

### swift-qwen3-tts_amd/csrc/engine_queue.cc

```cpp
#include "engine_stream.h"

namespace q3 {

ResolvedRequest Engine::check_queued(const q3tts_request& r, const q3tts_sampling& sp, const Voice* voice, bool open_text) const {
    const TalkerConfig& t = m_->cfg.talker;
    Q3_CHECK(r.ref_audio == nullptr, 3, "Invalid input: voice-clone requests (ref_audio) are not supported by q3tts_generate_queued");
    ResolvedRequest o = resolve(r, sp, voice);
    if (open_text) {
        Q3_CHECK(!o.clone, 3, "Invalid input: an open-text request cannot be a voice-clone request");
        o.n_tail = 0;
        o.text_open = true;
        o.open_max_tokens = r.max_tokens > 0 ? r.max_tokens : 2048;
        o.open_force_frames = sp.force_frames;
        o.max_frames = sp.force_frames > 0 ? sp.force_frames : o.open_max_tokens;
        o.target_token_count = int(o.text_ids.size()) - 3;
    }
    Q3_CHECK(m_->has_codec, 1, "Model not initialized: Speech tokenizer not loaded");
    Q3_CHECK(o.max_frames <= Fcap_, 3, "Invalid input: max_tokens exceeds the configured max_frames");
    Q3_CHECK(o.language_id < t.vocab_size && o.speaker_token < t.vocab_size, 3, "Invalid input: codec prefix id out of range");
    const int tl = int(o.text_ids.size());
    int nc = (o.language_id < 0 ? 3 : 4) + (o.speaker_token >= 0 ? 1 : 0) + 2;
    int np = int(o.instruct_ids.size()) + 3 + nc;
    int nt = (tl - o.n_tail > 4 ? tl - o.n_tail - 4 : 0) + 1;
    if (o.clone) {
// ... 668 lines not shown
        w.span = now - x.t0;
        w.codes.assign((size_t)(nf) * 16, 0);
        if (nf > 0)
            Q3_HIP(hipMemcpyAsync(w.codes.data(), e.codes_ + size_t(s) * e.Fcap_ * 16, size_t(nf) * 64, hipMemcpyDeviceToHost, e.st_));
        kvb += e.kv_bytes(x.np, nf);
        if (audio) retiring.push_back(s);
        x = QSlot{};
        any_retired = true;
    }
    if (any_retired) Q3_HIP(hipStreamSynchronize(e.st_));
    for (int s : retiring) audio->ss->retire(s, std::min(h_nframes[size_t(s)], e.Fcap_));
}

void Engine::QueueRun::loop() {
    Q3_HIP(hipEventRecord(e.ev_[2], e.st_));
    for (;;) {
        forget_settled();
        if (q.src->has_cancels()) apply_cancels();
        const int admitted = admit_boundary();
        if (open_text && q.src->has_appends()) e.apply_text_appends(q, sl, live);
        const BurstPlan p = burst_length(sl, burst_frames);
        if (p.runnable == 0) {
            if (!idle(p.running > 0)) break;
            continue;
        }
        launch_burst(p.burst, admitted);
        while_burst_runs();
        read_back(p.burst);
        if (audio) audio->feed();
        if (admitted) {
            float ms = 0;
            Q3_HIP(hipEventElapsedTime(&ms, e.ev_[0], e.ev_[1]));
            prefill_ms += ms;
        }
        retire();
    }
}

q3tts_timing Engine::QueueRun::finish() {
    Q3_HIP(hipEventRecord(e.ev_[3], e.st_));
    Q3_HIP(hipStreamSynchronize(e.st_));
    drain_decodes();
    q3tts_timing tm{};
    if (audio) {
        audio->zombies.clear();
        audio->ss->finish();
        audio->settle(true);
        audio->in_use.clear();
        codec_ms = audio->ss->codec_ms;
        tm.first_audio_ms = audio->ss->first_audio_ms;
        audio->redo_held(audio->ss->out);
    }
    float loop_ms = 0;
    Q3_HIP(hipEventElapsedTime(&loop_ms, e.ev_[2], e.ev_[3]));
    tm.prefill_ms = prefill_ms;
    tm.decode_ms = std::max(0.0, double(loop_ms) - prefill_ms);
    tm.codec_ms = codec_ms;
    tm.frame_steps = launched;
    tm.rows = served;
    tm.kv_bytes_read = kvb;
    tm.launches_per_frame_step = e.launches_per_step(S);
    return tm;
}

void Engine::run_queued(QueueShared& q, int S, const q3tts_sampling& sp, q3tts_event_cb cb, void* user) {
    Q3_HIP(hipSetDevice(m_->device));
    Q3_CHECK(S >= 1 && S <= Bm_, 3, "Invalid input: slots must be between 1 and max_batch");
    Q3_CHECK(!job_outstanding(), 3, "Invalid input: a q3tts_generate_begin job is outstanding (q3tts_generate_end must be called first)");
    ensure_queue_ws();
    if (q.voice_ref_max >= 0) extra_.grow(size_t(S) * (1 + q.voice_ref_max) * m_->cfg.talker.hidden_size);
    const double t_call = now_s();
    std::vector<int32_t> bt(size_t(S) * max_pages_);
    for (size_t i = 0; i < bt.size(); ++i) bt[i] = int32_t(i);
    Q3_HIP(hipMemcpyAsync(block_table_, bt.data(), bt.size() * 4, hipMemcpyHostToDevice, st_));
    for (int32_t* p : {kv_len_, cp_len_, n_frames_, max_frames_, trailing_idx_, n_trailing_, n_prompt_})
        Q3_HIP(hipMemsetAsync(p, 0, size_t(S) * 4, st_));
    Q3_HIP(hipMemsetAsync(row_key_, 0, size_t(S) * 4, st_));
    Q3_HIP(hipMemsetAsync(active_, 0, size_t(S), st_));
    Q3_HIP(hipMemsetAsync(finished_, 1, size_t(S), st_));
    q3tts_sampling call_wide = sp;
    call_wide.per_request = nullptr;
    upload_sampling(call_wide, 0u, S);
    build_cp_proj_tables();
    QueueRun run(*this, q, S, sp, cb, user, t_call);
    run.loop();
    timing = run.finish();
}

}
```

### swift-qwen3-tts_amd/csrc/kernels.h

```cpp
#pragma once
#include <hip/hip_runtime.h>

#include <cstdint>

namespace q3 {

struct DebugEnv {
    bool gemm_no_row_split;
    bool gemm_one_pair;
    bool gemm_parent_forms;
    bool no_tall_gemm;
    int tall_shape;
    int chunk_qsplit;
    bool conv_no_pw;
    bool nt_off;
    bool serial_jobs;
    bool fail_back_half;
    bool no_prefix_cache;
};
const DebugEnv& debug_env();
void debug_env_reload();

constexpr int kPageTokens = 64;
constexpr int kHeadDim = 128;

struct NormRowsArgs {
    const uint16_t* h;
    int hMB;
    const uint16_t* w;
    float eps;
    uint16_t* out;
    int outMB;
    float* ss_out;
    int M, H;
    const float* ss_in;
    int ss_count, ss_ld;
};
void launch_norm_rows(const NormRowsArgs& a, hipStream_t st);

struct GemmArgs {
    const uint16_t* W;
    const uint32_t* Wsb;
    const uint16_t* x;
    int xMB;
    int M, Mpad, N, K;
    int epi;
    uint16_t* y;
    int ldy;
    int y_tiled, yMB;
    const uint16_t* bias;
    int act_silu;
    const uint16_t* norm_w;
    const float* ss_in;
    int ss_count, ss_ld, norm_dim;
    float norm_eps;
    int nt_weights;
    int resid;
    float* ss_out;
};
void launch_gemm_skinny(const GemmArgs& a, hipStream_t st);
struct SkinnyGeom {
    bool tall;
    int split, mbw;
    int nw, ch, np;
    int gx;
    bool ntw;
    bool tm;
};
SkinnyGeom skinny_geometry(const GemmArgs& a);
bool launch_gemm_skinny_with_norm_rows(const GemmArgs& a, const NormRowsArgs& n, hipStream_t st);
bool gemm_norm_rows_rides(const GemmArgs& a, const NormRowsArgs& n);
bool launch_gemm_tall(const GemmArgs& a, hipStream_t st);
bool gemm_tall_takes(const GemmArgs& a);
int gemm_tall_shape(const GemmArgs& a);


struct AttnArgs {
    const uint16_t* qkv;
    int ld;
    const uint16_t* qn_w;
    const uint16_t* kn_w;
    float eps;
    const uint16_t* rope_cos;
    const uint16_t* rope_sin;
    uint16_t* kpool;
    uint16_t* vpool;
    const int32_t* block_table;
    int max_pages;
    const int32_t* kv_len;
    const uint8_t* active;
    uint16_t* out;
    int outMB;
    int n_heads, n_kv, B;
    float scale;
    int fixed_len;
    int identity_pages;
    int chunk;
    const int32_t* chunk_n_prompt;
    int chunk_r_base;
    int nt_kv;
};
void launch_attn_decode(const AttnArgs& a, hipStream_t st);

struct FrameEndArgs {
    const int32_t* cur_codes;
    const uint16_t* codec_emb;
    const uint16_t* const* cp_emb;
    const uint16_t* trailing;
    const int32_t* n_trailing;
    int32_t* trailing_idx;
    int Tmax;
    const uint16_t* tts_pad;
    uint16_t* h;
    int hMB, H, B, groups;
    float* ss_out;
    int32_t* n_frames;
    const int32_t* max_frames;
    uint8_t* finished;
    uint8_t* active;
    int32_t* cp_len;
    const uint8_t* text_open;
    uint8_t* starved;
};
void launch_frame_end(const FrameEndArgs& a, hipStream_t st);

struct SamplingParams {
    float temperature;
    int top_k;
    float top_p;
    float rep_penalty;
    uint64_t seed;
    uint32_t row0;
    int mask_eos;
};

struct SamplerArgs {
    const uint16_t* logits;
    int ldl, V;
    const SamplingParams* sp;
    int is_talker;
    int suppress_lo, suppress_hi, eos_id;
    uint8_t* seen;
    int cb;
    const int32_t* n_frames;
    const int32_t* max_frames;
    uint8_t* finished;
    uint8_t* active;
    int32_t* kv_len;
    int advance;
    const uint8_t* advance_gate;
    int32_t* cur_codes;
    int32_t* codes;
    int Fmax;
    const int32_t* forced;
    int forced_frames;
    int32_t* sampled;
    const uint16_t* emb;
    int emb_ld;
    uint16_t* next_x;
    int next_MB;
    int next_row0;
    float* next_ss;
    const float* emb_ss;
    int nss, next_ss_ld;
    int H;
    int B;
    uint16_t* logits_dump;
    int dump_ld, dump_off;
    const uint32_t* row_key;
};
void launch_sampler(const SamplerArgs& a, hipStream_t st);
void launch_sampler_with_frame_end(const SamplerArgs& a, const FrameEndArgs& fe, hipStream_t st);
void launch_ss_to_table(const float* ss, int ss_ld, float* dst, int nss, int rows, hipStream_t st);

void launch_gather_rows(const uint16_t* table, int ld, const int32_t* ids, const int32_t* token_map,
                        int n, int dim, uint16_t* out, int ldo, int out_MB, hipStream_t st);
void launch_tile_rows(const uint16_t* src, int lds, uint16_t* dst, int dstMB, int rows, int dim, hipStream_t st);
void launch_untile_rows(const uint16_t* src, int srcMB, uint16_t* dst, int ldd, int rows, int dim, hipStream_t st);
void launch_add_rows(const uint16_t* a, int lda, const uint16_t* b, int ldb, int rows, int dim,
                     uint16_t* out, int ldo, hipStream_t st);

struct PrefillLoadArgs {
    const uint16_t* prompt;
    const int32_t* n_prompt;
    int Pmax, step, H, B;
    uint16_t* h;
    int hMB;
    float* ss_out;
    uint8_t* active;
};
void launch_prefill_load(const PrefillLoadArgs& a, hipStream_t st);
void launch_advance_len(int32_t* kv_len, const uint8_t* active, int B, hipStream_t st);
void launch_stamp(unsigned long long* acc, unsigned long long* last, int k, hipStream_t st);
void launch_prefill_chunk_load(const PrefillLoadArgs& a, int C, hipStream_t st);
void launch_advance_len_chunk(int32_t* kv_len, const int32_t* n_prompt, int r_base, int C, int B, hipStream_t st);

struct AdmitDesc {
    int32_t slot, n_trailing, max_frames;
    uint32_t row_key;
    int32_t text_open;
    SamplingParams sp;
};
struct AdmitArgs {
    const AdmitDesc* desc;
    const uint16_t* src_h;
    int srcMB;
    const float* src_ss;
    const int32_t* src_kv_len;
    const int32_t* src_n_prompt;
    uint16_t* h;
    int hMB;
    float* ss;
    int H, V, Fmax, slots;
    int32_t *kv_len, *n_prompt, *n_trailing, *max_frames, *n_frames, *cp_len, *trailing_idx, *cur_codes, *codes;
    uint32_t* row_key;
    SamplingParams* sp;
    uint8_t *finished, *active, *seen;
    uint8_t *text_open, *starved;
};
void launch_admit_rows(const AdmitArgs& a, int k, hipStream_t st);
void launch_cancel_rows(uint64_t mask, uint8_t* finished, uint8_t* active, int slots, hipStream_t st);
struct TextAppendDesc {
    int32_t slot, src_row, n_new, close, max_frames, pad_;
};
struct TextAppendArgs {
    const TextAppendDesc* desc;
    const uint16_t* src;
    const uint16_t* eos_row;
    uint16_t* trailing;
    int32_t* n_trailing;
    uint8_t* text_open;
    int32_t* max_frames;
    int slots;
    FrameEndArgs fe;
};
void launch_text_append_rows(const TextAppendArgs& a, const TextAppendDesc* host, int k, hipStream_t st);


void launch_compose_rows(const uint16_t* proj, int ldp, const uint16_t* table, int ldt, const uint16_t* extra, int lde,
                         const int32_t* a, const int32_t* b, const int32_t* dst_row, uint16_t* dst, int ldd, int n, int dim,
                         hipStream_t st);
void launch_ref_embed_rows(const int32_t* codes, int T, int groups, const uint16_t* codec_emb, const uint16_t* const* cp_emb,
                           int H, uint16_t* out, int ldo, hipStream_t st);
void launch_f32_to_bf16(const float* x, uint16_t* out, int n, hipStream_t st);
struct DecodeRowDesc {
    const int32_t* ref;
    const int32_t* gen;
    int32_t Tref, F, dst_row, pad_;
};
void launch_build_decode_codes_rows(const DecodeRowDesc* host, const DecodeRowDesc* rows, int R, int32_t* out, int out_rows,
                                    int Fdec, hipStream_t st);

void launch_copy_rows(const uint16_t* src, int lds, uint16_t* dst, int ldd, int rows, int dim, hipStream_t st);

// ... 2 lines not shown
```

### swift-qwen3-tts_amd/csrc/kernels/sampler.hip

```cpp
#include "../common.h"
#include "../kernels.h"
#include "row_jobs.h"

namespace q3 {
namespace {

constexpr int kMaxVAll = 4096;

__device__ __forceinline__ void philox4x32_10(uint32_t c0, uint32_t c1, uint32_t c2, uint32_t c3, uint32_t k0,
                                              uint32_t k1, uint32_t (&out)[4]) {
#pragma unroll
    for (int r = 0; r < 10; ++r) {
        const uint64_t p0 = (uint64_t)0xD2511F53u * c0;
        const uint64_t p1 = (uint64_t)0xCD9E8D57u * c2;
        const uint32_t n0 = (uint32_t)(p1 >> 32) ^ c1 ^ k0;
        const uint32_t n1 = (uint32_t)p1;
        const uint32_t n2 = (uint32_t)(p0 >> 32) ^ c3 ^ k1;
        const uint32_t n3 = (uint32_t)p0;
        c0 = n0; c1 = n1; c2 = n2; c3 = n3;
        k0 += 0x9E3779B9u;
        k1 += 0xBB67AE85u;
    }
    out[0] = c0; out[1] = c1; out[2] = c2; out[3] = c3;
}

__device__ __forceinline__ float q3_logf(float x) {
    uint32_t u = __float_as_uint(x);
    int e = (int)((u >> 23) & 0xff) - 126;
    u = (u & 0x007fffffu) | 0x3f000000u;
    float m = __uint_as_float(u);
    if (m < 0.70710678118654752440f) {
        e -= 1;
        m = m + m;
    }
    const float f = m - 1.0f;
    const float z = f * f;
    float y = 7.0376836292E-2f;
    y = __fmaf_rn(y, f, -1.1514610310E-1f);
    y = __fmaf_rn(y, f, 1.1676998740E-1f);
    y = __fmaf_rn(y, f, -1.2420140846E-1f);
    y = __fmaf_rn(y, f, 1.4249322787E-1f);
    y = __fmaf_rn(y, f, -1.6668057665E-1f);
    y = __fmaf_rn(y, f, 2.0000714765E-1f);
    y = __fmaf_rn(y, f, -2.4999993993E-1f);
    y = __fmaf_rn(y, f, 3.3333331174E-1f);
    y = y * f;
    y = y * z;
    const float fe = (float)e;
    y = __fmaf_rn(fe, -2.12194440e-4f, y);
    y = __fmaf_rn(z, -0.5f, y);
    float r = f + y;
    r = __fmaf_rn(fe, 0.693359375f, r);
    return r;
}

__device__ __forceinline__ float q3_expf(float x) {
    if (x < -87.0f) return 0.0f;
    if (x > 88.0f) return INFINITY;
    const float fx = floorf(__fmaf_rn(x, 1.44269504088896341f, 0.5f));
    float r = __fmaf_rn(fx, -0.693359375f, x);
    r = __fmaf_rn(fx, 2.12194440e-4f, r);
    const float z = r * r;
    float y = 1.9875691500E-4f;
    y = __fmaf_rn(y, r, 1.3981999507E-3f);
    y = __fmaf_rn(y, r, 8.3334519073E-3f);
    y = __fmaf_rn(y, r, 4.1665795894E-2f);
    y = __fmaf_rn(y, r, 1.6666665459E-1f);
    y = __fmaf_rn(y, r, 5.0000001201E-1f);
    y = __fmaf_rn(y, z, r);
    y = y + 1.0f;
    const int n = (int)fx;
    return y * __uint_as_float((uint32_t)(n + 127) << 23);
}

__device__ __forceinline__ float gumbel_noise(uint64_t seed, uint32_t row, uint32_t draw, uint32_t i) {
    uint32_t r[4];
    philox4x32_10(i, row, draw, 0u, (uint32_t)seed, (uint32_t)(seed >> 32), r);
    const float u = ((float)(r[0] >> 8) + 0.5f) * 5.9604644775390625e-08f;
    return -q3_logf(-q3_logf(u));
}

__device__ __forceinline__ uint32_t key16(float v) {
    const uint32_t u = __float_as_uint(v) >> 16;
    return (u & 0x8000u) ? (~u & 0xffffu) : (u | 0x8000u);
}

struct Best {
    float v;
    int i;
};
__device__ __forceinline__ Best better(Best a, Best b) {
    return (b.v > a.v || (b.v == a.v && b.i < a.i)) ? b : a;
}

template <int O>
__device__ __forceinline__ Best partner(Best x) {
    Best y;
    const float fi = __int_as_float(x.i);
    if constexpr (O == 32 || O == 16) {
        float a, b, c, d;
        if constexpr (O == 32) { XorPartner::swap32(x.v, a, b); XorPartner::swap32(fi, c, d); }
        else { XorPartner::swap16(x.v, a, b); XorPartner::swap16(fi, c, d); }
        const bool upper = O == 32 ? ((threadIdx.x & 32) != 0) : ((threadIdx.x & 16) != 0);
        y.v = upper ? a : b;
        y.i = __float_as_int(upper ? c : d);
    } else if constexpr (O == 8) {
        y.v = XorPartner::x8(x.v); y.i = __float_as_int(XorPartner::x8(fi));
    } else if constexpr (O == 4) {
        y.v = XorPartner::x4(x.v); y.i = __float_as_int(XorPartner::x4(fi));
    } else if constexpr (O == 2) {
        y.v = XorPartner::x2(x.v); y.i = __float_as_int(XorPartner::x2(fi));
    } else {
        y.v = XorPartner::x1(x.v); y.i = __float_as_int(XorPartner::x1(fi));
    }
    return y;
}

template <int kThreads>
__device__ Best block_argmax(Best x, Best* scratch) {
    x = better(x, partner<32>(x));
    x = better(x, partner<16>(x));
    x = better(x, partner<8>(x));
    x = better(x, partner<4>(x));
    x = better(x, partner<2>(x));
    x = better(x, partner<1>(x));
    const int wave = threadIdx.x >> 6;
    __syncthreads();
    if ((threadIdx.x & 63) == 0) scratch[wave] = x;
    __syncthreads();
    Best r = scratch[0];
    for (int w = 1; w < kThreads / 64; ++w) r = better(r, scratch[w]);
    return r;
}

template <int kThreads, int kMaxV, bool TALKER, bool FEND>
__device__ __forceinline__ void sampler_body(const SamplerArgs& a, const FrameEndArgs* fe) {
    constexpr int kElems = kMaxV / kThreads;
    __builtin_amdgcn_s_setprio(3);
    __shared__ float vals[kMaxV];
    __shared__ uint32_t sortbuf[kMaxV];
    __shared__ float sval[kMaxV];
    __shared__ int n_surv;
    __shared__ uint32_t hist[2][256];
    __shared__ Best scratch[kThreads / 64];
    __shared__ uint32_t wcount[kElems][kThreads / 64];
    __shared__ int sel[2][2];

    const int b = blockIdx.x, tid = threadIdx.x;
    const int V = a.V;
    const uint16_t* lrow = a.logits + (size_t)b * a.ldl;
    uint16_t raw[kElems];
    uint8_t was_seen[kElems];
    const bool want_seen = TALKER && a.seen;
#pragma unroll
    for (int k = 0; k < kElems; ++k) {
        const int i = k * kThreads + tid;
        const int ic = i < V ? i : V - 1;
        raw[k] = lrow[ic];
        was_seen[k] = want_seen ? a.seen[(size_t)b * V + ic] : (uint8_t)0;
    }
    const SamplingParams sp = a.sp[b];
    const bool row_done = a.finished[b] != 0;
    const int frame = a.n_frames[b];
    const uint8_t gate_raw = *(a.advance_gate ? a.advance_gate + b : a.finished + b);
    const uint32_t key_raw = *(a.row_key ? a.row_key + b : reinterpret_cast<const uint32_t*>(a.n_frames) + b);
    const uint32_t row_key = a.row_key ? key_raw : sp.row0 + (uint32_t)b;
    const bool gate = a.advance_gate ? (gate_raw != 0) : true;
    if (tid < 256) {
        hist[0][tid] = 0;
        hist[1][tid] = 0;
    }
    if (tid == 0) n_surv = 0;
    if (row_done) {
        if (tid == 0 && a.advance && gate && !a.advance_gate) a.kv_len[b] += 1;
        if constexpr (FEND)
            if (tid == 0) fe->cp_len[b] = 0;
        return;
    }
    if (a.logits_dump && frame < a.forced_frames)
        for (int i = tid; i < V; i += kThreads)
            a.logits_dump[((size_t)b * a.forced_frames + frame) * a.dump_ld + a.dump_off + i] = lrow[i];

    const bool use_top_p = sp.top_p > 0.f && sp.top_p < 1.0f;
    const bool need_vals = TALKER || use_top_p;
    const float pen = rbf(sp.rep_penalty);
    const bool use_pen = want_seen && sp.rep_penalty != 1.0f;
    float l[kElems];
#pragma unroll
    for (int k = 0; k < kElems; ++k) {
        const int i = k * kThreads + tid;
        float v = -INFINITY;
        if (i < V) {
            v = bf2f(raw[k]);
            if (TALKER) {
                if (i >= a.suppress_lo && i < a.suppress_hi && i != a.eos_id) v = -INFINITY;
                if (sp.mask_eos && i == a.eos_id) v = -INFINITY;
                if (use_pen && was_seen[k]) v = (v < 0.f) ? rbf(v * pen) : rbf(v / pen);
            }
        }
        l[k] = v;
        if (need_vals) vals[k * kThreads + tid] = v;
    }
    __syncthreads();

    int tok;
    if (sp.temperature <= 0.f) {
        Best x{-INFINITY, 0x7fffffff};
#pragma unroll
        for (int k = 0; k < kElems; ++k) {
            const int i = k * kThreads + tid;
            if (i < V) x = better(x, Best{l[k], i});
        }
        const Best g = block_argmax<kThreads>(x, scratch);
        tok = g.i;
        if (tok == 0x7fffffff || g.v == -INFINITY) tok = 0;
    } else {
        const bool have_eos = TALKER && a.eos_id >= 0 && a.eos_id < V;
        const float eos_logit = have_eos ? vals[a.eos_id] : 0.f;
        if (sp.top_k > 0 && sp.top_k < V) {
            uint32_t key[kElems];
#pragma unroll
            for (int k = 0; k < kElems; ++k) key[k] = key16(l[k]);
            int need = sp.top_k;
            uint32_t prefix = 0;
            for (int level = 0; level < 2; ++level) {
#pragma unroll
                for (int k = 0; k < kElems; ++k) {
                    const int i = k * kThreads + tid;
                    if (i < V && (level == 0 || (key[k] >> 8) == prefix))
                        atomicAdd(&hist[level][level == 0 ? (key[k] >> 8) : (key[k] & 0xff)], 1u);
                }
                __syncthreads();
                if (tid < 64) {
                    const uint32_t* hl = hist[level];
                    const uint32_t h0 = hl[4 * tid], h1 = hl[4 * tid + 1], h2 = hl[4 * tid + 2], h3 = hl[4 * tid + 3];
                    const int own = (int)(h0 + h1 + h2 + h3);
                    int suf = own;
#pragma unroll
                    for (int o = 1; o < 64; o <<= 1) {
                        const int v = __shfl_down(suf, o, 64);
                        if (tid + o < 64) suf += v;
                    }
                    const int above = suf - own;
                    const bool mine = above < need && suf >= need;
                    const bool none = __ballot(mine) == 0ull;
                    if (mine) {
                        int cum = above, bin = 4 * tid + 3;
                        const int hh[4] = {(int)h0, (int)h1, (int)h2, (int)h3};
                        for (; bin > 4 * tid; --bin) {
                            if (cum + hh[bin & 3] >= need) break;
                            cum += hh[bin & 3];
                        }
                        sel[level][0] = bin;
                        sel[level][1] = need - cum;
                    }
                    if (none && tid == 0) {
                        sel[level][0] = 0;
                        sel[level][1] = need - (suf - (int)h0);
                    }
                }
                __syncthreads();
                if (level == 0) prefix = (uint32_t)sel[0][0];
                else prefix = (prefix << 8) | (uint32_t)sel[1][0];
                need = sel[level][1];
            }
            const uint32_t kt = prefix;
            unsigned long long bal[kElems];
            {
                const int lane = tid & 63, wave = tid >> 6;
#pragma unroll
                for (int k = 0; k < kElems; ++k) {
                    const int i = k * kThreads + tid;
                    bal[k] = __ballot((i < V) && key[k] == kt);
                    if (lane == 0) wcount[k][wave] = (uint32_t)__popcll(bal[k]);
                }
                __syncthreads();
                int base = 0;
#pragma unroll
                for (int k = 0; k < kElems; ++k) {
                    const int i = k * kThreads + tid;
                    const bool eq = (i < V) && key[k] == kt;
                    const int below = __popcll(bal[k] & ((1ull << lane) - 1ull));
                    int woff = 0, total = 0;
                    for (int w = 0; w < kThreads / 64; ++w) {
                        if (w < wave) woff += (int)wcount[k][w];
                        total += (int)wcount[k][w];
                    }
                    const int rank = base + woff + below;
                    if (i < V && (key[k] < kt || (eq && rank >= need))) l[k] = -INFINITY;
                    base += total;
                }
            }
            if (use_top_p) {
#pragma unroll
                for (int k = 0; k < kElems; ++k) vals[k * kThreads + tid] = l[k];
                __syncthreads();
            }
        }
        if (use_top_p) {
            const int lane = tid & 63;
#pragma unroll
            for (int k = 0; k < kElems; ++k) {
                const int i = k * kThreads + tid;
                const bool keep = i < V && l[k] != -INFINITY;
                const unsigned long long bal = __ballot(keep);
                int base = 0;
                if (lane == 0 && bal) base = atomicAdd(&n_surv, __popcll(bal));
                base = __shfl(base, 0, 64);
                if (keep) sortbuf[base + __popcll(bal & ((1ull << lane) - 1ull))] = (key16(l[k]) << 16) | (uint32_t)i;
            }
            __syncthreads();
            const int nf = n_surv;
            int P = 2;
            while (P < nf) P <<= 1;
            for (int q = nf + tid; q < P; q += kThreads) sortbuf[q] = 0xffffffffu;
            __syncthreads();
            for (int size = 2; size <= P; size <<= 1) {
                for (int stride = size >> 1; stride > 0; stride >>= 1) {
                    for (int t = tid; t < P / 2; t += kThreads) {
                        const int lo = 2 * t - (t & (stride - 1));
                        const int hi = lo + stride;
                        const bool up = ((lo & size) == 0);
                        const uint32_t x = sortbuf[lo], y = sortbuf[hi];
                        if ((x > y) == up) {
                            sortbuf[lo] = y;
                            sortbuf[hi] = x;
                        }
                    }
                    __syncthreads();
                }
            }
            for (int r = tid; r < nf; r += kThreads) sval[r] = rbf(q3_expf(vals[sortbuf[r] & 0xffffu]));
            __syncthreads();
            if (tid == 0) {
                const float thr = rbf(1.0f - sp.top_p);
                float run = 0.f;
                for (int r = 0; r < nf; ++r) {
                    run += sval[r];
                    if (!(rbf(run) > thr)) vals[sortbuf[r] & 0xffffu] = -INFINITY;
                }
                n_surv = 0;
            }
            __syncthreads();
#pragma unroll
            for (int k = 0; k < kElems; ++k) l[k] = vals[k * kThreads + tid];
        }
        if (have_eos && !sp.mask_eos) {
#pragma unroll
            for (int k = 0; k < kElems; ++k)
                if (k * kThreads + tid == a.eos_id) l[k] = eos_logit;
        }
        const float invt = rbf(1.0f / sp.temperature);
        const uint32_t draw = (uint32_t)frame * 16u + (uint32_t)a.cb;
#pragma unroll
        for (int k = 0; k < kElems; ++k) {
            const int i = k * kThreads + tid;
            if (i < V && l[k] != -INFINITY) {
                const int slot = atomicAdd(&n_surv, 1);
                sortbuf[slot] = (uint32_t)i;
                sval[slot] = l[k];
            }
        }
        __syncthreads();
        const int ns = n_surv;
        Best x{-INFINITY, 0x7fffffff};
        for (int q = tid; q < ns; q += kThreads) {
            const int i = (int)sortbuf[q];
            const float v = rbf(sval[q] * invt) + gumbel_noise(sp.seed, row_key, draw, (uint32_t)i);
            x = better(x, Best{v, i});
        }
        Best r = block_argmax<kThreads>(x, scratch);
        tok = (r.i == 0x7fffffff) ? 0 : r.i;
    }

    int used = tok;
    if (a.forced && frame < a.forced_frames) used = a.forced[((size_t)b * a.forced_frames + frame) * 16 + a.cb];
    if (tid == 0) {
        if (a.sampled && frame < a.forced_frames) a.sampled[((size_t)b * a.forced_frames + frame) * 16 + a.cb] = tok;
        a.cur_codes[(size_t)b * 16 + a.cb] = used;
        if (TALKER) {
            if (a.seen && used >= 0 && used < V) a.seen[(size_t)b * V + used] = 1;
            if (a.advance && a.active[b]) a.kv_len[b] += 1;
            if (used == a.eos_id) {
                a.finished[b] = 1;
                a.active[b] = 0;
            } else if (frame < a.Fmax) {
                a.codes[((size_t)b * a.Fmax + frame) * 16] = used;
            }
        } else {
            if (a.advance && gate) a.kv_len[b] += 1;
            if (frame < a.Fmax) a.codes[((size_t)b * a.Fmax + frame) * 16 + a.cb] = used;
        }
    }
    if (a.next_x) {
        const uint4* src = reinterpret_cast<const uint4*>(a.emb + (size_t)used * a.emb_ld);
        float ss = 0.f;
        for (int i = tid; i < a.H / 8; i += kThreads) {
            const uint4 v = src[i];
            const uint32_t w[4] = {v.x, v.y, v.z, v.w};
#pragma unroll
            for (int j = 0; j < 4; ++j) ss += lo_bf(w[j]) * lo_bf(w[j]) + hi_bf(w[j]) * hi_bf(w[j]);
            *reinterpret_cast<uint4*>(a.next_x + act_tiled_offset(b + a.next_row0, 8 * i, a.next_MB)) = v;
        }
        if (a.emb_ss) {
            for (int j = tid; j < a.nss; j += kThreads)
                a.next_ss[(size_t)j * a.next_ss_ld + b + a.next_row0] = a.emb_ss[(size_t)used * a.nss + j];
        } else if (a.next_ss) {
            ss = wave_sum(ss);
            __syncthreads();
            if ((tid & 63) == 0) vals[tid >> 6] = ss;
            __syncthreads();
            if (tid == 0) {
                float t = 0.f;
                for (int w = 0; w < kThreads / 64; ++w) t += vals[w];
                a.next_ss[b] = t;
            }
        }
    }
    if constexpr (FEND) {
        __shared__ float fe_sh[4];
        frame_end_job(*fe, b, tid, used, fe_sh);
    }
}

template <int kThreads, int kMaxV, bool TALKER>
__global__ __launch_bounds__(kThreads) void sampler_kernel(SamplerArgs a) {
    sampler_body<kThreads, kMaxV, TALKER, false>(a, nullptr);
}
struct SamplerFendArgs {
    SamplerArgs s;
    FrameEndArgs fe;
};
__global__ __launch_bounds__(1024) void sampler_fend_kernel(SamplerFendArgs a) {
    sampler_body<1024, 2048, false, true>(a.s, &a.fe);
}

}

void launch_sampler_with_frame_end(const SamplerArgs& a, const FrameEndArgs& fe, hipStream_t st) {
    Q3_CHECK(!a.is_talker && a.V <= 2048, 3, "sampler: the end-of-frame rider belongs to a code-predictor draw");
    SamplerFendArgs s{a, fe};
    hipLaunchKernelGGL(sampler_fend_kernel, dim3(a.B), dim3(1024), 0, st, s);
}

void launch_sampler(const SamplerArgs& a, hipStream_t st) {
    Q3_CHECK(a.V <= kMaxVAll, 3, "sampler: vocabulary larger than 4096 is not supported");
    if (!a.is_talker && a.V <= 2048) hipLaunchKernelGGL((sampler_kernel<1024, 2048, false>), dim3(a.B), dim3(1024), 0, st, a);
    else if (a.is_talker) hipLaunchKernelGGL((sampler_kernel<1024, 4096, true>), dim3(a.B), dim3(1024), 0, st, a);
    else hipLaunchKernelGGL((sampler_kernel<1024, 4096, false>), dim3(a.B), dim3(1024), 0, st, a);
}

}
```

### swift-qwen3-tts_amd/csrc/model.h

```cpp
#pragma once
#include <memory>
#include <mutex>
#include <string>
#include <vector>

#include "config.h"
#include "safetensors.h"

namespace q3 {

struct LinearW {
    const uint16_t* w = nullptr;
    const uint32_t* sb = nullptr;
    const uint16_t* bias = nullptr;
    int N = 0, K = 0;
    int Np = 0, Kp = 0;
};

struct LayerW {
    const uint16_t* ln1 = nullptr;
    const uint16_t* ln2 = nullptr;
    const uint16_t* qn = nullptr;
    const uint16_t* kn = nullptr;
    LinearW qkv;
// ... 76 lines not shown
        SnakeW snake;
        ConvW tconv;
        int stride = 1, Cout = 0;
        Res res[3];
    };
    std::vector<Block> blocks;
    SnakeW out_snake;
    bool f16_main = false;
    const float* out_w = nullptr;
    const float* out_b = nullptr;
    int out_C = 0;
};

struct CodecEncW {
    const float* init_w = nullptr;
    const float* init_b = nullptr;
    int init_C = 0, init_K = 0;
    struct Layer {
        ConvW res1, res2;
        ConvW down;
        int ratio = 1, C = 0;
    };
    std::vector<Layer> layers;
    ConvW final_conv;
    struct TLayer {
        const float *ln1_w = nullptr, *ln1_b = nullptr, *ln2_w = nullptr, *ln2_b = nullptr;
        ConvW qkv, o, fc1, fc2;
    };
    std::vector<TLayer> tlayers;
    int heads = 0, hidden = 0;
    const float* rope_cos = nullptr;
    const float* rope_sin = nullptr;
    int max_T = 0;
    ConvW down;
    int ds = 2;
    ConvW rvq_in;
    int dim = 0, bins = 0, n_layers = 0;
    std::vector<const float*> cb, c2;
    const float* const* cb_dev = nullptr;
    const float* const* c2_dev = nullptr;
};

struct SpeakerEncW {
    ConvW dft;
    const float* mel_fb = nullptr;
    int n_fft = 1024, hop = 256, nfreq = 513, n_mels = 128;
    ConvW b0;
    struct Block {
        ConvW tdnn1, tdnn2, se1, se2;
        std::vector<ConvW> res;
        int C = 0;
    };
    Block blocks[3];
    ConvW mfa, asp_tdnn, asp_conv, fc;
    int scale = 8, enc_dim = 0;
};

struct Model {
    ModelConfig cfg;
    int device = 0;
    uint8_t* arena = nullptr;
    size_t arena_bytes = 0;

    StackW talker, cp;
    const uint16_t* codec_emb = nullptr;
    const uint16_t* text_emb = nullptr;
    const int32_t* token_map = nullptr;
    int64_t text_emb_rows = 0;
    LinearW fc1, fc2, codec_head, cp_proj;
    bool has_cp_proj = false;
    std::vector<LinearW> lm_head;
    std::vector<const uint16_t*> cp_emb;
    const uint16_t* const* cp_emb_dev = nullptr;
    bool has_codec = false;
    CodecW codec;
    bool has_codec_encoder = false;
    CodecEncW codec_enc;
    bool has_speaker_encoder = false;
    SpeakerEncW speaker;
    int64_t step_weight_bytes = 0;
    std::vector<void*> side_allocs;
    mutable std::vector<const uint16_t*> cp_pe;
    mutable std::vector<const float*> cp_pss;
    mutable std::vector<void*> lazy_allocs;
    mutable std::mutex lazy_mutex;

    ~Model();
};

struct LoadOptions {
    int device = 0;
    int max_pos_talker = 4096;
    bool skip_tensor_data = false;
};

std::unique_ptr<Model> load_model(const std::string& dir, const LoadOptions& opt);

void launch_tile_weights(const uint16_t* src, int N, int K, uint16_t* dst, int KC, int tile_off, int tile_stride,
                         hipStream_t st, int rows_per_tile = 16, int row_off = 0);
void launch_tile_int4(const uint32_t* wq, const uint16_t* scales, const uint16_t* biases, int N, int K, void* dq,
                      uint32_t* dsb, int KC, int tile_off, int tile_stride, hipStream_t st, int rows_per_tile = 16, int row_off = 0);

}
```

### swift-qwen3-tts_amd/qwen3tts/_lib.py

```python
from __future__ import annotations

import ctypes as C
import os

_HERE = os.path.dirname(os.path.abspath(__file__))
LIB_PATH = os.environ.get("Q3TTS_LIB") or os.path.join(_HERE, "libq3tts_hip.so")

u16p = C.POINTER(C.c_uint16)
i32p = C.POINTER(C.c_int32)
f32p = C.POINTER(C.c_float)
u8p = C.POINTER(C.c_uint8)


class LoadOpts(C.Structure):
    _fields_ = [("device", C.c_int32), ("max_batch", C.c_int32), ("max_frames", C.c_int32),
                ("max_prompt", C.c_int32), ("use_graph", C.c_int32), ("weights_from_broadcast", C.c_int32),
                ("n_streams", C.c_int32), ("codec_overlap_cus", C.c_int32), ("codec_fp32", C.c_int32),
                ("output_sample_rate", C.c_int32), ("speed", C.c_float), ("request_speeds", C.c_int32)]


class LoadOptsEx(C.Structure):
    _fields_ = [("base", LoadOpts), ("pitch", C.c_float)]


# ... 193 lines not shown

_lib = None


def lib() -> C.CDLL:
    global _lib
    if _lib is not None:
        return _lib
    if not os.path.exists(LIB_PATH):
        raise RuntimeError(f"{LIB_PATH} is missing: build the HIP engine first "
                           "(make -C swift-qwen3-tts_amd); there is no CPU fallback")
    L = C.CDLL(LIB_PATH)
    vp = C.c_void_p
    L.q3tts_default_load_opts.argtypes = [C.POINTER(LoadOpts)]
    L.q3tts_default_sampling.argtypes = [C.POINTER(Sampling)]
    L.q3tts_model_load.argtypes = [C.c_char_p, C.POINTER(LoadOpts), C.POINTER(vp)]
    L.q3tts_model_free.argtypes = [vp]
    L.q3tts_model_free.restype = None
    L.q3tts_last_error.argtypes = [vp]
    L.q3tts_last_error.restype = C.c_char_p
    L.q3tts_model_arena.argtypes = [vp, C.POINTER(vp), C.POINTER(C.c_size_t)]
    L.q3tts_model_get_info.argtypes = [vp, C.POINTER(ModelInfo)]
    L.q3tts_comm_get_unique_id.argtypes = [C.POINTER(CommId)]
    L.q3tts_model_broadcast.argtypes = [vp, C.POINTER(CommId), C.c_int32, C.c_int32, C.c_int32]
    L.q3tts_model_arena_checksum.argtypes = [vp, C.POINTER(C.c_uint64)]
    L.q3tts_model_num_speakers.argtypes = [vp]
    L.q3tts_model_speaker_name.argtypes = [vp, C.c_int32]
    L.q3tts_model_speaker_name.restype = C.c_char_p
    L.q3tts_generate.argtypes = [vp, C.POINTER(Request), C.c_int32, C.POINTER(Sampling), EVENT_CB, vp,
                                 C.POINTER(Result)]
    L.q3tts_generate_queued.argtypes = [vp, C.POINTER(Request), C.c_int32, C.c_int32, C.POINTER(Sampling), EVENT_CB, vp,
                                        C.POINTER(Result)]
    L.q3tts_voice_create.argtypes = [vp, f32p, C.c_int64, i32p, C.c_int32, C.POINTER(vp)]
    if hasattr(L, "q3tts_resample"):
        L.q3tts_voice_create_rate.argtypes = [vp, f32p, C.c_int64, C.c_int32, i32p, C.c_int32, C.POINTER(vp)]
        L.q3tts_resample.argtypes = [vp, f32p, C.c_int64, C.c_int32, C.c_int32, C.c_int32, f32p, C.c_int64, C.POINTER(C.c_int64)]
    if hasattr(L, "q3tts_time_stretch"):
        L.q3tts_model_get_speed.argtypes = [vp, C.POINTER(C.c_float), C.POINTER(C.c_int32), C.POINTER(C.c_int32)]
        L.q3tts_time_stretch.argtypes = [vp, f32p, C.c_int64, C.c_float, C.c_int32, f32p, C.c_int64, C.POINTER(C.c_int64)]
    L.q3tts_voice_free.argtypes = [vp, vp]
    L.q3tts_voice_free.restype = None
    L.q3tts_voice_get_info.argtypes = [vp, C.POINTER(VoiceInfo)]
    L.q3tts_generate_voices.argtypes = [vp, C.POINTER(Request), C.POINTER(vp), C.c_int32, C.POINTER(Sampling), EVENT_CB, vp,
                                        C.POINTER(Result)]
    L.q3tts_generate_queued_voices.argtypes = [vp, C.POINTER(Request), C.POINTER(vp), C.c_int32, C.c_int32, C.POINTER(Sampling),
                                               EVENT_CB, vp, C.POINTER(Result)]
    if hasattr(L, "q3tts_session_open"):
        L.q3tts_session_open.argtypes = [vp, C.POINTER(SessionOpts), C.POINTER(Sampling), EVENT_CB, vp, C.POINTER(vp)]
        L.q3tts_session_submit.argtypes = [vp, C.POINTER(Request), vp, C.POINTER(RowSampling), C.POINTER(C.c_int64)]
        L.q3tts_session_cancel.argtypes = [vp, C.c_int64]
        L.q3tts_session_wait.argtypes = [vp, C.c_int64, C.c_int32, C.POINTER(Result), i32p]
        L.q3tts_session_get_stats.argtypes = [vp, C.POINTER(SessionStats)]
        L.q3tts_session_close.argtypes = [vp, C.c_int32]
    if hasattr(L, "q3tts_session_submit_open"):
        L.q3tts_session_submit_open.argtypes = [vp, C.POINTER(Request), C.POINTER(RowSampling), C.POINTER(C.c_int64)]
        L.q3tts_session_append_text.argtypes = [vp, C.c_int64, i32p, C.c_int32, C.c_int32]
        L.q3tts_session_get_text_stats.argtypes = [vp, C.POINTER(SessionTextStats)]
        L.q3tts_debug_text_resume.argtypes = [vp, C.c_int32, C.c_int32, u16p, i32p, u16p, u16p, f32p, i32p]
    L.q3tts_generate_begin.argtypes = [vp, C.POINTER(Request), C.c_int32, C.POINTER(Sampling), EVENT_CB, vp, C.c_int32, C.POINTER(vp)]
    L.q3tts_generate_end.argtypes = [vp, vp, C.POINTER(Result)]
    L.q3tts_pcm_to_int16.argtypes = [f32p, C.c_int64, C.POINTER(C.c_int16)]
    L.q3tts_pcm_to_int16.restype = None
    L.q3tts_write_wav.argtypes = [C.c_char_p, f32p, C.c_int64, C.c_int32]
    L.q3tts_result_free.argtypes = [C.POINTER(Result), C.c_int32]
    L.q3tts_result_free.restype = None
    L.q3tts_codec_decode.argtypes = [vp, i32p, i32p, C.c_int32, C.c_int32, f32p, C.POINTER(C.c_int64)]
    L.q3tts_codec_decode_streamed.argtypes = [vp, i32p, i32p, C.c_int32, C.c_int32, C.c_int32, C.c_int32, C.c_int32, f32p]
    if hasattr(L, "q3tts_codec_decode_streamed_prefixed"):
        L.q3tts_codec_decode_streamed_prefixed.argtypes = [vp, i32p, i32p, i32p, C.c_int32, C.c_int32, C.c_int32, C.c_int32, C.c_int32,
                                                           f32p]
    if hasattr(L, "q3tts_request_speed_info"):
        L.q3tts_request_speed_info.argtypes = [vp, C.c_float, C.POINTER(C.c_float), i32p, i32p, i32p]
        L.q3tts_debug_stretch_rows.argtypes = [vp, f32p, i32p, i32p, C.c_int32, C.c_int64, f32p, C.c_int64]
    if hasattr(L, "q3tts_pitch_shift"):
        L.q3tts_default_load_opts_ex.argtypes = [C.POINTER(LoadOptsEx)]
        L.q3tts_default_load_opts_ex.restype = None
        L.q3tts_model_load_ex.argtypes = [C.c_char_p, C.POINTER(LoadOptsEx), C.POINTER(vp)]
        L.q3tts_model_get_pitch.argtypes = [vp, C.POINTER(C.c_float), i32p, i32p, i32p]
        L.q3tts_pitch_shift.argtypes = [vp, f32p, C.c_int64, C.c_float, f32p, C.c_int64, C.POINTER(C.c_int64)]
        L.q3tts_debug_resample_ratio.argtypes = [vp, f32p, i32p, C.c_int32, C.c_int64, C.c_int64, C.c_int64, C.c_int32, C.c_int32, C.c_int32,
                                                 f32p, C.c_int64]
    if hasattr(L, "q3tts_debug_prefix_states"):
        L.q3tts_debug_prefix_states.argtypes = [vp, i32p, C.POINTER(C.c_int64), C.POINTER(C.c_int64)]
    if hasattr(L, "q3tts_debug_codec_stream_slots"):
        L.q3tts_debug_codec_stream_slots.argtypes = [vp, i32p, i32p, C.c_int32, C.c_int32, C.c_int32, C.c_int32, C.c_int32, C.c_int32,
                                                     C.c_int32, f32p]
    L.q3tts_debug_set_codec_scratch.argtypes = [C.c_uint64]
    L.q3tts_debug_set_codec_scratch.restype = None
    L.q3tts_debug_reload_env.argtypes = []
    L.q3tts_debug_reload_env.restype = None
    L.q3tts_last_timing.argtypes = [vp, C.POINTER(Timing)]
    L.q3tts_codec_encode.argtypes = [vp, f32p, C.c_int64, i32p, C.c_int32, i32p]
    L.q3tts_codec_encoded_frames.argtypes = [vp, C.c_int64]
    L.q3tts_speaker_embedding.argtypes = [vp, f32p, C.c_int64, C.c_int32, f32p, C.c_int32]
    L.q3tts_debug_frontend_stage.argtypes = [vp, f32p, C.c_int64, C.c_char_p, f32p, C.c_int64, i32p, i32p]
    L.q3tts_tokenizer_load.argtypes = [C.c_char_p, C.POINTER(vp)]
    L.q3tts_tokenizer_free.argtypes = [vp]
    L.q3tts_tokenizer_free.restype = None
    L.q3tts_tokenizer_encode.argtypes = [vp, C.c_char_p, i32p, C.c_int32, i32p]
    L.q3tts_debug_prepare_inputs.argtypes = [vp, C.POINTER(Request), u16p, C.c_int32, i32p, u16p, C.c_int32,
                                             i32p, u16p]
    L.q3tts_debug_generate_forced.argtypes = [vp, C.POINTER(Request), C.c_int32, C.POINTER(Sampling), i32p,
                                              C.c_int32, u16p, u16p, i32p]
    L.q3tts_debug_sample.argtypes = [vp, u16p, C.c_int32, C.c_int32, C.POINTER(Sampling), u8p, C.c_int32,
                                     C.c_int32, C.c_int32, C.c_uint32, C.c_uint32, i32p]
    L.q3tts_debug_linear.argtypes = [vp, u16p, u16p, u16p, C.c_int32, C.c_int32, C.c_int32, u16p]
    L.q3tts_debug_attention.argtypes = [vp, C.POINTER(AttnDebug)]
    if hasattr(L, "q3tts_debug_gemm"):
        L.q3tts_debug_gemm.argtypes = [vp, C.POINTER(GemmDebug)]
    if hasattr(L, "q3tts_debug_conv"):
        L.q3tts_debug_conv.argtypes = [vp, C.POINTER(ConvDebug)]
    if hasattr(L, "q3tts_debug_rowop"):
        L.q3tts_debug_rowop.argtypes = [vp, C.POINTER(RowopDebug)]
    if hasattr(L, "q3tts_debug_lmop"):
        L.q3tts_debug_lmop.argtypes = [vp, C.POINTER(LmopDebug)]
    if hasattr(L, "q3tts_debug_build_decode_codes"):
        L.q3tts_debug_build_decode_codes.argtypes = [vp, i32p, i32p, i32p, i32p, C.c_int32, C.c_int32, C.c_int32, C.c_int32, i32p]
    L.q3tts_debug_codec_stage.argtypes = [vp, i32p, C.c_int32, C.c_char_p, f32p, C.c_int64, i32p, i32p]
    _lib = L
    return L


GEOM_FIELDS = ("rode", "tall", "tall_shape", "split", "mbw", "nw", "ch", "np", "gx", "ntw", "tm")


def gemm_geometry(**kw) -> dict:
    a = GemmDebug(geometry_only=1, **kw)
    st = lib().q3tts_debug_gemm(None, C.byref(a))
    if st != 0:
        raise ValueError("q3tts_debug_gemm refused the arguments (status %d): %r" % (st, kw))
    return {f: int(getattr(a, f)) for f in GEOM_FIELDS}


CONV_GEOM_FIELDS = ("family", "BN", "pro", "pw_depth", "KT", "X32", "CT2", "PT", "wdb", "grid_x", "grid_y", "grid_z", "lds_bytes")
CONV_OPERANDS = ("x2", "bias", "bias2", "scale", "snake", "act2", "post", "res", "out", "out2", "w2", "pcm", "nonfinite")


def conv_geometry(frames=None, **kw) -> dict:
    ops = {k: kw.pop(k, False) for k in CONV_OPERANDS}
    a = ConvDebug(geometry_only=1, **kw)
    one = (C.c_float * 4)()
    fp = C.cast(one, f32p)
    a.w = fp
    for name in ("x2", "bias", "bias2", "scale", "w2", "pcm"):
        if ops[name]:
            setattr(a, name, fp)
    for name in ("snake", "act2", "post"):
        if ops[name]:
            setattr(a, name + "_alpha", fp)
            setattr(a, name + "_beta", fp)
    for name in ("res", "out", "out2"):
        if ops[name]:
            setattr(a, name, C.cast(one, C.c_void_p))
    if ops["nonfinite"]:
        a.nonfinite = C.cast(one, i32p)
    fr = None
    if frames is not None:
        fr = (C.c_int32 * len(frames))(*frames)
        a.frames = C.cast(fr, i32p)
    st = lib().q3tts_debug_conv(None, C.byref(a))
    if st != 0:
        raise ValueError("q3tts_debug_conv refused the arguments (status %d): %r" % (st, kw))
    return {f: int(getattr(a, f)) for f in CONV_GEOM_FIELDS}


def reload_debug_env() -> None:
# ... 2 lines not shown
```

### swift-qwen3-tts_amd/qwen3tts/model.py

```python
from __future__ import annotations

import ctypes as C
import math
import os
from dataclasses import dataclass
from typing import Callable, Iterator, List, Optional, Sequence, Tuple

import numpy as np

from . import _lib as L


class Qwen3TTSError(RuntimeError):

    def __init__(self, status: int, message: str):
        super().__init__(message)
        self.status = status


@dataclass
class AudioGenerationInfo:
    prompt_token_count: int
    generation_token_count: int
    prefill_time: float
# ... 541 lines not shown
        yield from events

    def generate_voice_clone(self, text: Optional[str] = None, reference_audio: Optional[np.ndarray] = None,
                             reference_text: Optional[str] = None, language: str = "auto", temperature: float = 0.9,
                             top_k: int = 50, top_p: float = 1.0, repetition_penalty: float = 1.5,
                             max_tokens: int = 2048, *, seed: int = 0, text_ids: Optional[Sequence[int]] = None,
                             ref_text_ids: Optional[Sequence[int]] = None,
                             target_token_count: Optional[int] = None, sample_rate: Optional[int] = None) -> np.ndarray:
        if sample_rate is not None and int(sample_rate) != 24000:
            reference_audio = self.resample(reference_audio, int(sample_rate), 24000, centred=True)
        if text_ids is None:
            if self.tokenizer is None:
                raise Qwen3TTSError(1, "Model not initialized: Tokenizer not loaded")
            t = chat_template_ids(self.tokenizer, text)
            text_ids, target_token_count = t["text_ids"], t["target_token_count"]
            ref_text_ids = self.tokenizer(f"<|im_start|>assistant\n{reference_text}<|im_end|>\n")
        req = GenerationRequest(text_ids, int(target_token_count or 0), None, None, language, max_tokens,
                                ref_audio=reference_audio, ref_text_ids=ref_text_ids)
        r = self.generate_batch([req], temperature, top_k, top_p, repetition_penalty, seed)[0]
        if r.status != 0:
            raise Qwen3TTSError(r.status, "Generation failed: No tokens generated")
        return r.audio

    def codec_encode(self, audio: np.ndarray) -> np.ndarray:
        a = np.ascontiguousarray(np.asarray(audio, np.float32).reshape(-1))
        cap = max(1, int(self._lib.q3tts_codec_encoded_frames(self._h, a.size)))
        codes = np.zeros((16, cap), np.int32)
        n = C.c_int32(0)
        self._check(self._lib.q3tts_codec_encode(self._h, a.ctypes.data_as(L.f32p), a.size, codes.ctypes.data_as(L.i32p),
                                                 cap, C.byref(n)))
        return codes.reshape(-1)[: 16 * n.value].reshape(16, n.value)

    def extract_speaker_embedding(self, audio: np.ndarray, sample_rate: int = 24000) -> np.ndarray:
        a = np.ascontiguousarray(np.asarray(audio, np.float32).reshape(-1))
        out = np.zeros(max(1, self.info.speaker_embedding_dim), np.float32)
        self._check(self._lib.q3tts_speaker_embedding(self._h, a.ctypes.data_as(L.f32p), a.size, sample_rate,
                                                      out.ctypes.data_as(L.f32p), out.size))
        return out

    def debug_frontend_stage(self, audio: np.ndarray, stage: str, cap_floats: int = 1 << 26) -> np.ndarray:
        a = np.ascontiguousarray(np.asarray(audio, np.float32).reshape(-1))
        out = np.zeros(cap_floats, np.float32)
        T, Cc = C.c_int32(0), C.c_int32(0)
        self._check(self._lib.q3tts_debug_frontend_stage(self._h, a.ctypes.data_as(L.f32p), a.size, stage.encode(),
                                                         out.ctypes.data_as(L.f32p), out.size, C.byref(T), C.byref(Cc)))
        return out[: T.value * Cc.value].reshape(T.value, Cc.value).copy()

    def codec_decode(self, codes: np.ndarray, n_frames: Optional[Sequence[int]] = None):
        codes = np.ascontiguousarray(codes, np.int32)
        if codes.ndim == 2:
            codes = codes[None]
        B, F, _ = codes.shape
        nf = np.ascontiguousarray(n_frames if n_frames is not None else [F] * B, np.int32)
        up = self.info.samples_per_frame
        pcm = np.zeros((B, F * up), np.float32)
        lens = np.zeros(B, np.int64)
        self._check(self._lib.q3tts_codec_decode(self._h, codes.ctypes.data_as(L.i32p), nf.ctypes.data_as(L.i32p), B, F,
                                                 pcm.ctypes.data_as(L.f32p), lens.ctypes.data_as(C.POINTER(C.c_int64))))
        return pcm, lens

    def codec_decode_streamed(self, codes: np.ndarray, chunk_frames: int, window: int, lookahead: int = 4,
                              n_frames: Optional[Sequence[int]] = None) -> np.ndarray:
        codes = np.ascontiguousarray(codes, np.int32)
        if codes.ndim == 2:
            codes = codes[None]
        B, F, G = codes.shape
        nf = np.asarray(n_frames if n_frames is not None else [F] * B, np.int32)
        pcm = np.zeros((B, F * self.info.samples_per_frame), np.float32)
        self._check(self._lib.q3tts_codec_decode_streamed(self._h, codes.ctypes.data_as(L.i32p), nf.ctypes.data_as(L.i32p), B, F,
                                                          chunk_frames, window, lookahead, pcm.ctypes.data_as(L.f32p)))
        return pcm

    def codec_decode_streamed_prefixed(self, codes: np.ndarray, n_prefix: Sequence[int], n_frames: Sequence[int], chunk_frames: int,
                                       window: int, lookahead: int = 4) -> np.ndarray:
        codes = np.ascontiguousarray(codes, np.int32)
        B, F, G = codes.shape
        npre, nf = np.asarray(n_prefix, np.int32), np.asarray(n_frames, np.int32)
        assert npre.shape == (B,) and nf.shape == (B,) and G == 16
        pcm = np.zeros((B, max(int(nf.max()), 0) * self.info.samples_per_frame), np.float32)
        self._check(self._lib.q3tts_codec_decode_streamed_prefixed(self._h, codes.ctypes.data_as(L.i32p), npre.ctypes.data_as(L.i32p),
                                                                   nf.ctypes.data_as(L.i32p), B, F, int(chunk_frames), int(window),
                                                                   int(lookahead), pcm.ctypes.data_as(L.f32p)))
        return pcm

    def debug_prefix_states(self) -> Tuple[int, int, int]:
        n, b, r = C.c_int32(0), C.c_int64(0), C.c_int64(0)
        self._check(self._lib.q3tts_debug_prefix_states(self._h, C.byref(n), C.byref(b), C.byref(r)))
        return n.value, b.value, r.value

    def debug_codec_stream_slots(self, codes: np.ndarray, n_frames: Sequence[int], slots: int, burst: int, chunk_frames: int,
                                 window: int, lookahead: int) -> np.ndarray:
        codes = np.ascontiguousarray(codes, np.int32)
        N, F, G = codes.shape
        nf = np.asarray(n_frames, np.int32)
        assert nf.shape == (N,) and G == 16
        pcm = np.zeros((N, F * self.info.samples_per_frame), np.float32)
        self._check(self._lib.q3tts_debug_codec_stream_slots(self._h, codes.ctypes.data_as(L.i32p), nf.ctypes.data_as(L.i32p), N, F,
                                                             int(slots), int(burst), int(chunk_frames), int(window), int(lookahead),
                                                             pcm.ctypes.data_as(L.f32p)))
        return pcm

    def debug_prepare_inputs(self, req: GenerationRequest):
        arr, keep = self._marshal([req])
        H = self.info.hidden_size
        cap = 1024
        ie = np.zeros((cap, H), np.uint16)
        tr = np.zeros((cap, H), np.uint16)
        pad = np.zeros((H,), np.uint16)
        n1, n2 = C.c_int32(), C.c_int32()
        self._check(self._lib.q3tts_debug_prepare_inputs(self._h, arr, ie.ctypes.data_as(L.u16p), cap, C.byref(n1),
                                                         tr.ctypes.data_as(L.u16p), cap, C.byref(n2),
                                                         pad.ctypes.data_as(L.u16p)))
        del keep
        return ie[: n1.value].copy(), tr[: n2.value].copy(), pad

    def debug_generate_forced(self, reqs: Sequence[GenerationRequest], forced_codes: np.ndarray, temperature=0.0,
                              top_k=50, top_p=1.0, repetition_penalty=1.05, seed=0, row_base=0):
        arr, keep = self._marshal(reqs)
        n = len(reqs)
        forced = np.ascontiguousarray(forced_codes, np.int32).reshape(n, -1, 16)
        F = forced.shape[1]
        V, Vc, G = self.info.vocab_size, self.info.cp_vocab_size, self.info.num_code_groups
        tl = np.zeros((n, F, V), np.uint16)
        cl = np.zeros((n, F, G - 1, Vc), np.uint16)
        sampled = np.zeros((n, F, 16), np.int32)
        s = self._sampling(temperature, top_k, top_p, repetition_penalty, seed, 0, row_base=row_base, reqs=reqs)
        self._check(self._lib.q3tts_debug_generate_forced(
            self._h, arr, n, C.byref(s), forced.ctypes.data_as(L.i32p), F, tl.ctypes.data_as(L.u16p),
            cl.ctypes.data_as(L.u16p), sampled.ctypes.data_as(L.i32p)))
        del keep
        return tl, cl, sampled

    def debug_sample(self, logits: np.ndarray, temperature=0.9, top_k=50, top_p=1.0, repetition_penalty=1.0,
                     seed=0, seen: Optional[np.ndarray] = None, suppress=(0, 0), eos_id=-1, row0=0, draw=0,
                     mask_eos=False, per_row: Optional[Sequence[Optional[RequestSampling]]] = None):
        logits = np.ascontiguousarray(logits, np.uint16)
        rows, V = logits.shape
        s = self._sampling(temperature, top_k, top_p, repetition_penalty, seed, 1 if mask_eos else 0)
        if per_row is not None:
            assert len(per_row) == rows
            s._rows = self._row_sampling(per_row)
            if s._rows is not None:
                s.per_request = C.cast(s._rows, C.POINTER(L.RowSampling))
        toks = np.zeros(rows, np.int32)
        sp = np.ascontiguousarray(seen, np.uint8).ctypes.data_as(L.u8p) if seen is not None else None
        self._check(self._lib.q3tts_debug_sample(self._h, logits.ctypes.data_as(L.u16p), rows, V, C.byref(s), sp,
                                                 suppress[0], suppress[1], eos_id, row0, draw,
                                                 toks.ctypes.data_as(L.i32p)))
        return toks

    def debug_text_resume(self, tables: np.ndarray, codes, text_row: np.ndarray):
        tables = np.ascontiguousarray(tables, np.uint16)
        _, V, H = tables.shape
        codes = np.ascontiguousarray(codes, np.int32)
        text_row = np.ascontiguousarray(text_row, np.uint16)
        assert tables.shape[0] == 16 and codes.shape == (16,) and text_row.shape == (H,)
        h, ss, state = np.zeros((3, H), np.uint16), np.zeros(3, np.float32), np.zeros((3, 8), np.int32)
        self._check(self._lib.q3tts_debug_text_resume(self._h, H, V, tables.ctypes.data_as(L.u16p), codes.ctypes.data_as(L.i32p),
                                                      text_row.ctypes.data_as(L.u16p), h.ctypes.data_as(L.u16p),
                                                      ss.ctypes.data_as(L.f32p), state.ctypes.data_as(L.i32p)))
        return h, ss, state

    def debug_linear(self, x: np.ndarray, W: np.ndarray, bias: Optional[np.ndarray] = None) -> np.ndarray:
        x = np.ascontiguousarray(x, np.uint16)
        W = np.ascontiguousarray(W, np.uint16)
        M, K = x.shape
# ... 286 lines not shown
```

Before: 10610.

## Precompute code-predictor layer-0 QKV rows per codebook token into lookup tables

In the code predictor, the first layer's input comes from a sampled token's embedding, so its normed QKV projection depends only on the token. This builds a table of layer-0 QKV outputs for every vocab entry of the first eight codebook tables. When the sampler picks a token it copies that row into the QKV buffer, and the first layer's QKV GEMM is skipped. It costs a one-time build and extra device memory, and adds a row copy inside the sampler. Some sampler timeline instrumentation is also added behind a compile flag.

```diff
diff --git a/include/q3tts.h b/include/q3tts.h
--- a/include/q3tts.h
+++ b/include/q3tts.h
@@ -433,6 +433,9 @@
 
 q3tts_status q3tts_debug_prefix_states(q3tts_model* m, int32_t* n_states, int64_t* device_bytes, int64_t* n_restored);
 
+q3tts_status q3tts_debug_cp_qkv_rows(q3tts_model* m, int32_t table, const int32_t* codes, int32_t n, uint16_t* stored,
+                                     uint16_t* rebuilt, uint16_t* pass, int32_t* ld);
+
 q3tts_status q3tts_debug_stretch_rows(q3tts_model* m, const float* x, const int32_t* lens, const int32_t* hops, int32_t B,
                                       int64_t x_stride, float* y, int64_t y_stride);
 
diff --git a/swift-qwen3-tts_amd/csrc/api.cc b/swift-qwen3-tts_amd/csrc/api.cc
--- a/swift-qwen3-tts_amd/csrc/api.cc
+++ b/swift-qwen3-tts_amd/csrc/api.cc
@@ -662,6 +662,16 @@
     });
 }
 
+q3tts_status q3tts_debug_cp_qkv_rows(q3tts_model* m, int32_t table, const int32_t* codes, int32_t n, uint16_t* stored, uint16_t* rebuilt,
+                                     uint16_t* pass, int32_t* ld) {
+    return guarded(m, [&] {
+        Q3_CHECK(m && codes && ld && (!stored || (rebuilt && pass)), 3, "Invalid input: null argument");
+        int l = 0;
+        m->eng->lane0().debug_cp_qkv_rows(table, codes, n, stored, rebuilt, pass, &l);
+        *ld = l;
+    });
+}
+
 q3tts_status q3tts_debug_text_resume(q3tts_model* m, int32_t H, int32_t V, const uint16_t* tables, const int32_t* codes,
                                      const uint16_t* text_row, uint16_t* out_h, float* out_ss, int32_t* out_state) {
     return guarded(m, [&] {
diff --git a/swift-qwen3-tts_amd/csrc/debug_env.cc b/swift-qwen3-tts_amd/csrc/debug_env.cc
--- a/swift-qwen3-tts_amd/csrc/debug_env.cc
+++ b/swift-qwen3-tts_amd/csrc/debug_env.cc
@@ -29,6 +29,7 @@
     d->serial_jobs = number("Q3TTS_SERIAL_JOBS", 0) != 0;
     d->fail_back_half = number("Q3TTS_TEST_FAIL_BACK_HALF", 0) != 0;
     d->no_prefix_cache = number("Q3TTS_NO_PREFIX_CACHE", 0) != 0;
+    d->cp_qkv_tables = number("Q3TTS_CP_QKV_TABLES", kCpQkvTablesDefault);
     return d;
 }
 }
diff --git a/swift-qwen3-tts_amd/csrc/engine.cc b/swift-qwen3-tts_amd/csrc/engine.cc
--- a/swift-qwen3-tts_amd/csrc/engine.cc
+++ b/swift-qwen3-tts_amd/csrc/engine.cc
@@ -165,6 +165,58 @@
         Q3_HIP(hipStreamSynchronize(st_));
     }
     cp_tables_ = true;
+}
+
+SamplerArgs Engine::cp_next_input_args(int table) const {
+    const TalkerConfig& t = m_->cfg.talker;
+    const int H = t.hidden_size, CH = t.cp.hidden_size, MBL = Mp_ / 16;
+    SamplerArgs sc{};
+    sc.emb = m_->cp_emb[size_t(table)]; sc.emb_ld = H; sc.H = H; sc.next_MB = MBL;
+    sc.next_x = m_->has_cp_proj ? cp_x_ : cp_.h;
+    sc.next_ss = m_->has_cp_proj ? nullptr : cp_.ss_a;
+    if (cp_tables_) {
+        sc.emb = m_->cp_pe[size_t(table)]; sc.emb_ld = CH; sc.H = CH; sc.next_x = cp_.h;
+        sc.emb_ss = m_->cp_pss[size_t(table)]; sc.nss = CH / 16; sc.next_ss = cp_.ss_a; sc.next_ss_ld = Mp_;
+    }
+    if (table < cp_qkv_tables_) {
+        sc.qkv_tab = m_->cp_qkv + size_t(table) * size_t(t.cp.vocab_size) * size_t(cp_.ld_qkv);
+        sc.qkv_out = cp_.qkv; sc.qkv_ld = cp_.ld_qkv;
+    }
+    return sc;
+}
+
+void Engine::enqueue_cp_qkv_rows(SamplerArgs g, int c0, const int32_t* codes, int rows) {
+    g.B = rows;
+    g.qkv_tab = nullptr; g.qkv_out = nullptr; g.qkv_ld = 0;
+    launch_sampler_next_input(g, c0, codes, st_);
+    launch_gemm_skinny(layer_qkv_args(m_->cp, cp_, 0, rows, m_->has_cp_proj ? m_->cp.hidden / 16 : 1, true, 0), st_);
+}
+
+void Engine::build_cp_qkv_tables() {
+    if (cp_qkv_tables_ > 0) return;
+    const TalkerConfig& t = m_->cfg.talker;
+    const int CH = m_->cp.hidden, Vc = t.cp.vocab_size, ld = cp_.ld_qkv;
+    const int ntab = std::min(debug_env().cp_qkv_tables, t.num_code_groups - 2);
+    if (ntab <= 0 || CH > 2048 || m_->cp.layers.empty() || (m_->has_cp_proj && !cp_tables_) || ld % 8 != 0) return;
+    std::lock_guard<std::mutex> lock(m_->lazy_mutex);
+    if (!m_->cp_qkv) {
+        uint16_t* tab = nullptr;
+        Q3_HIP(hipMalloc(reinterpret_cast<void**>(&tab), size_t(ntab) * Vc * ld * 2));
+        m_->lazy_allocs.push_back(tab);
+        const int step = std::min(Mp_, 64);
+        for (int i = 0; i < ntab; ++i) {
+            SamplerArgs g = cp_next_input_args(i);
+            for (int c0 = 0; c0 < Vc; c0 += step) {
+                const int rows = std::min(step, Vc - c0);
+                enqueue_cp_qkv_rows(g, c0, nullptr, rows);
+                Q3_HIP(hipMemcpyAsync(tab + (size_t(i) * Vc + c0) * ld, cp_.qkv, size_t(rows) * ld * 2, hipMemcpyDeviceToDevice, st_));
+            }
+        }
+        Q3_HIP(hipStreamSynchronize(st_));
+        m_->cp_qkv = tab;
+        m_->cp_qkv_ntab = ntab;
+    }
+    cp_qkv_tables_ = m_->cp_qkv_ntab;
 }
 
 void Engine::alloc_workspace() {
@@ -251,9 +303,20 @@
     return a;
 }
 
+GemmArgs Engine::layer_qkv_args(const StackW& s, const Stream& w, size_t l, int M, int ss_count_in, bool prologue, int ntw) const {
+    const LayerW& L = s.layers[l];
+    GemmArgs q = gemm_args(L.qkv, prologue ? w.h : w.xn, M);
+    q.epi = 0; q.y = w.qkv; q.ldy = w.ld_qkv; q.nt_weights = ntw;
+    if (prologue) {
+        q.norm_w = L.ln1; q.ss_in = w.ss_a; q.ss_count = (l == 0) ? ss_count_in : s.hidden / 16; q.norm_dim = s.hidden; q.norm_eps = s.eps;
+    }
+    return q;
+}
+
 void Engine::enqueue_layers(const StackW& s, Stream& w, int B, uint16_t* kpool, uint16_t* vpool, size_t layer_stride,
                             const int32_t* block_table, int max_pages, const int32_t* kv_len, const uint8_t* active,
-                            int ss_count_in, int fixed_len, int chunk, const int32_t* chunk_n_prompt, int chunk_r_base) {
+                            int ss_count_in, int fixed_len, int chunk, const int32_t* chunk_n_prompt, int chunk_r_base,
+                            bool qkv0_given) {
     const int H = s.hidden, MBL = Mp_ / 16, tiles = H / 16;
     const int M = B * (chunk > 1 ? chunk : 1);
     Q3_CHECK(M <= Mp_, 7, "internal error: chunk does not fit the activation buffers");
@@ -271,12 +334,10 @@
     };
     for (size_t l = 0; l < s.layers.size(); ++l) {
         const LayerW& L = s.layers[l];
+        const bool have_qkv = qkv0_given && l == 0;
+        Q3_CHECK(!have_qkv || (prologue_qkv && chunk <= 1), 7, "internal error: q/k/v tables outside the norm-prologue decode form");
         if (!prologue_qkv) norm_into_xn(L.ln1, w.ss_a, (l == 0) ? ss_count_in : tiles);
-        GemmArgs q = gemm_args(L.qkv, prologue_qkv ? w.h : w.xn, M);
-        q.epi = 0; q.y = w.qkv; q.ldy = w.ld_qkv; q.nt_weights = ntw;
-        if (prologue_qkv) {
-            q.norm_w = L.ln1; q.ss_in = w.ss_a; q.ss_count = (l == 0) ? ss_count_in : tiles; q.norm_dim = H; q.norm_eps = s.eps;
-        }
+        const GemmArgs q = layer_qkv_args(s, w, l, M, ss_count_in, prologue_qkv, ntw);
         AttnArgs at{};
         at.qkv = w.qkv; at.ld = w.ld_qkv; at.qn_w = L.qn; at.kn_w = L.kn; at.eps = s.eps;
         at.rope_cos = s.rope_cos; at.rope_sin = s.rope_sin;
@@ -287,7 +348,7 @@
         at.chunk = chunk; at.chunk_n_prompt = chunk_n_prompt; at.chunk_r_base = chunk_r_base;
         at.scale = powf(float(kHeadDim), -0.5f);
         at.nt_kv = ntkv;
-        launch_gemm_skinny(q, counted());
+        if (!have_qkv) launch_gemm_skinny(q, counted());
         launch_attn_decode(at, counted());
         GemmArgs o = gemm_args(L.o, w.ao, M);
         o.epi = 3; o.y = w.h; o.yMB = MBL; o.resid = 1; o.ss_out = w.ss_b; o.nt_weights = ntw;
@@ -310,7 +371,7 @@
     enqueue_layers(m_->talker, tk_, B, kpool_, vpool_, kv_layer_stride_, block_table_, max_pages_, kv_len_, active_, 1, -1, 1, nullptr, 0);
 }
 
-void Engine::enqueue_cp_pass(int B, bool from_talker, int head, int cp_pos, bool projected) {
+void Engine::enqueue_cp_pass(int B, bool from_talker, int head, int cp_pos, bool projected, bool qkv0_given) {
     const TalkerConfig& t = m_->cfg.talker;
     const int H = t.hidden_size, CH = m_->cp.hidden, MBL = Mp_ / 16;
     int ss_count = 1;
@@ -331,7 +392,8 @@
     } else if (from_talker) {
         talker_norm_into(cp_.h, cp_.ss_a);
     }
-    enqueue_layers(m_->cp, cp_, B, cp_kpool_, cp_vpool_, cp_kv_layer_stride_, cp_block_table_, 1, cp_len_, nullptr, ss_count, cp_pos, 1, nullptr, 0);
+    enqueue_layers(m_->cp, cp_, B, cp_kpool_, cp_vpool_, cp_kv_layer_stride_, cp_block_table_, 1, cp_len_, nullptr, ss_count, cp_pos, 1, nullptr, 0,
+                   qkv0_given);
 }
 
 FrameEndArgs Engine::frame_end_args(int B) const {
@@ -419,7 +481,7 @@
         const bool second_of_pair = pair && i == 0;
         const int Mh = second_of_pair ? 2 * B : B;
         if (!second_of_pair) {
-            enqueue_cp_pass(B, false, i, i + 1, cp_tables_ && i >= 1);
+            enqueue_cp_pass(B, false, i, i + 1, cp_tables_ && i >= 1, i >= 1 && i <= cp_qkv_tables_);
             stamp(5);
         }
         {
@@ -436,13 +498,12 @@
         sc.cur_codes = cur_codes_; sc.codes = codes_; sc.Fmax = Fcap_;
         sc.forced = dbg ? forced_dev_ : nullptr; sc.forced_frames = dbg ? dbg->frames : 0;
         sc.sampled = dbg ? sampled_dev_ : nullptr;
+        sc.H = H; sc.B = B;
         if (i + 1 < groups - 1) {
-            sc.emb = m_->cp_emb[size_t(i)]; sc.emb_ld = H; sc.next_x = next_x; sc.next_MB = MBL; sc.next_ss = next_ss;
-        }
-        sc.H = H; sc.B = B;
-        if (cp_tables_ && i + 1 < groups - 1) {
-            sc.emb = m_->cp_pe[size_t(i)]; sc.emb_ld = CH; sc.H = CH; sc.next_x = cp_.h;
-            sc.emb_ss = m_->cp_pss[size_t(i)]; sc.nss = CH / 16; sc.next_ss = cp_.ss_a; sc.next_ss_ld = Mp_;
+            const SamplerArgs ni = cp_next_input_args(i);
+            sc.emb = ni.emb; sc.emb_ld = ni.emb_ld; sc.H = ni.H; sc.next_x = ni.next_x; sc.next_MB = ni.next_MB; sc.next_ss = ni.next_ss;
+            sc.emb_ss = ni.emb_ss; sc.nss = ni.nss; sc.next_ss_ld = ni.next_ss_ld;
+            sc.qkv_tab = ni.qkv_tab; sc.qkv_out = ni.qkv_out; sc.qkv_ld = ni.qkv_ld;
         }
         sc.logits_dump = (dbg && dbg->cp_logits) ? cl_dump_ : nullptr; sc.dump_ld = (groups - 1) * Vc; sc.dump_off = i * Vc;
         sc.row_key = frame_row_key_;
@@ -1354,6 +1415,7 @@
     const int n = J.n;
     const bool use_graph = opts_.use_graph && !dbg;
     build_cp_proj_tables();
+    build_cp_qkv_tables();
     hipGraphExec_t ge = use_graph ? frame_graph(n) : nullptr;
     int frames_cap = 0;
     for (auto& r : rr) frames_cap = std::max(frames_cap, r.max_frames);
diff --git a/swift-qwen3-tts_amd/csrc/engine.h b/swift-qwen3-tts_amd/csrc/engine.h
--- a/swift-qwen3-tts_amd/csrc/engine.h
+++ b/swift-qwen3-tts_amd/csrc/engine.h
@@ -190,6 +190,7 @@
                               uint16_t* trailing, int cap_trailing, int* n_trailing, uint16_t* tts_pad);
     void debug_sample(const uint16_t* logits, int rows, int V, const q3tts_sampling& sp, const uint8_t* seen,
                       int suppress_lo, int suppress_hi, int eos_id, uint32_t row0, uint32_t draw, int32_t* tokens);
+    void debug_cp_qkv_rows(int table, const int32_t* codes, int n, uint16_t* stored, uint16_t* rebuilt, uint16_t* pass, int* ld);
     void debug_text_resume(int H, int V, const uint16_t* tables, const int32_t* codes, const uint16_t* text, uint16_t* out_h,
                            float* out_ss, int32_t* out_state);
     void debug_linear(const uint16_t* x, const uint16_t* W, const uint16_t* bias, int M, int K, int N, uint16_t* y);
@@ -263,6 +264,11 @@
     uint16_t* cp_x2_ = nullptr;
     bool cp_tables_ = false;
     void build_cp_proj_tables();
+    int cp_qkv_tables_ = 0;
+    void build_cp_qkv_tables();
+    void enqueue_cp_qkv_rows(SamplerArgs g, int c0, const int32_t* codes, int rows);
+    SamplerArgs cp_next_input_args(int table) const;
+    GemmArgs layer_qkv_args(const StackW& s, const Stream& w, size_t l, int M, int ss_count_in, bool prologue, int ntw) const;
     float* cp_ss2_ = nullptr;
     uint16_t *kpool_ = nullptr, *vpool_ = nullptr, *cp_kpool_ = nullptr, *cp_vpool_ = nullptr;
     size_t kv_layer_stride_ = 0, cp_kv_layer_stride_ = 0;
@@ -433,9 +439,10 @@
     void project_rows(const std::vector<int32_t>& ids, int rows);
     void enqueue_layers(const StackW& s, Stream& w, int B, uint16_t* kpool, uint16_t* vpool, size_t layer_stride,
                         const int32_t* block_table, int max_pages, const int32_t* kv_len, const uint8_t* active,
-                        int ss_count_in, int fixed_len, int chunk, const int32_t* chunk_n_prompt, int chunk_r_base);
+                        int ss_count_in, int fixed_len, int chunk, const int32_t* chunk_n_prompt, int chunk_r_base,
+                        bool qkv0_given = false);
     void enqueue_talker_step(int B, bool with_head);
-    void enqueue_cp_pass(int B, bool from_talker, int head, int cp_pos, bool projected = false);
+    void enqueue_cp_pass(int B, bool from_talker, int head, int cp_pos, bool projected = false, bool qkv0_given = false);
     void enqueue_frame(int B, const DebugOpts* dbg);
     FrameEndArgs frame_end_args(int B) const;
     hipGraphExec_t frame_graph(int B);
diff --git a/swift-qwen3-tts_amd/csrc/engine_debug.cc b/swift-qwen3-tts_amd/csrc/engine_debug.cc
--- a/swift-qwen3-tts_amd/csrc/engine_debug.cc
+++ b/swift-qwen3-tts_amd/csrc/engine_debug.cc
@@ -77,6 +77,32 @@
     Q3_HIP(hipMemcpy(cc.data(), cur_codes_, cc.size() * 4, hipMemcpyDeviceToHost));
     for (int r = 0; r < rows; ++r) tokens[r] = cc[size_t(r) * 16];
     Q3_HIP(hipMemset(seen_, 0, size_t(rows) * V));
+}
+
+void Engine::debug_cp_qkv_rows(int table, const int32_t* codes, int n, uint16_t* stored, uint16_t* rebuilt, uint16_t* pass, int* ld_out) {
+    build_cp_proj_tables();
+    build_cp_qkv_tables();
+    const TalkerConfig& t = m_->cfg.talker;
+    const int Vc = t.cp.vocab_size, ld = cp_.ld_qkv;
+    *ld_out = ld;
+    Q3_CHECK(cp_qkv_tables_ > 0, 3, "debug_cp_qkv_rows: this configuration has no q/k/v tables (or Q3TTS_CP_QKV_TABLES=0)");
+    Q3_CHECK(table >= 0 && table < cp_qkv_tables_ && n >= 1 && n <= std::min(Bm_, 64), 3, "debug_cp_qkv_rows: table / n out of range");
+    for (int j = 0; j < n; ++j) Q3_CHECK(codes[j] >= 0 && codes[j] < Vc, 3, "debug_cp_qkv_rows: a code outside the table");
+    if (!stored) return;
+    const SamplerArgs g = cp_next_input_args(table);
+    const uint16_t* tab = m_->cp_qkv + size_t(table) * Vc * ld;
+    const int step = std::min(Mp_, 64);
+    for (int j = 0; j < n; ++j) {
+        Q3_HIP(hipMemcpy(stored + size_t(j) * ld, tab + size_t(codes[j]) * ld, size_t(ld) * 2, hipMemcpyDeviceToHost));
+        const int c0 = codes[j] / step * step;
+        enqueue_cp_qkv_rows(g, c0, nullptr, std::min(step, Vc - c0));
+        Q3_HIP(hipStreamSynchronize(st_));
+        Q3_HIP(hipMemcpy(rebuilt + size_t(j) * ld, cp_.qkv + size_t(codes[j] - c0) * ld, size_t(ld) * 2, hipMemcpyDeviceToHost));
+    }
+    Q3_HIP(hipMemcpy(cur_codes_, codes, size_t(n) * 4, hipMemcpyHostToDevice));
+    enqueue_cp_qkv_rows(g, 0, cur_codes_, n);
+    Q3_HIP(hipStreamSynchronize(st_));
+    Q3_HIP(hipMemcpy(pass, cp_.qkv, size_t(n) * ld * 2, hipMemcpyDeviceToHost));
 }
 
 void Engine::debug_linear(const uint16_t* x, const uint16_t* W, const uint16_t* bias, int M, int K, int N, uint16_t* y) {
diff --git a/swift-qwen3-tts_amd/csrc/engine_queue.cc b/swift-qwen3-tts_amd/csrc/engine_queue.cc
--- a/swift-qwen3-tts_amd/csrc/engine_queue.cc
+++ b/swift-qwen3-tts_amd/csrc/engine_queue.cc
@@ -774,6 +774,7 @@
     call_wide.per_request = nullptr;
     upload_sampling(call_wide, 0u, S);
     build_cp_proj_tables();
+    build_cp_qkv_tables();
     QueueRun run(*this, q, S, sp, cb, user, t_call);
     run.loop();
     timing = run.finish();
diff --git a/swift-qwen3-tts_amd/csrc/kernels.h b/swift-qwen3-tts_amd/csrc/kernels.h
--- a/swift-qwen3-tts_amd/csrc/kernels.h
+++ b/swift-qwen3-tts_amd/csrc/kernels.h
@@ -17,7 +17,9 @@
     bool serial_jobs;
     bool fail_back_half;
     bool no_prefix_cache;
-};
+    int cp_qkv_tables;
+};
+constexpr int kCpQkvTablesDefault = 8;
 const DebugEnv& debug_env();
 void debug_env_reload();
 
@@ -168,8 +170,12 @@
     uint16_t* logits_dump;
     int dump_ld, dump_off;
     const uint32_t* row_key;
+    const uint16_t* qkv_tab;
+    uint16_t* qkv_out;
+    int qkv_ld;
 };
 void launch_sampler(const SamplerArgs& a, hipStream_t st);
+void launch_sampler_next_input(const SamplerArgs& a, int code0, const int32_t* codes, hipStream_t st);
 void launch_sampler_with_frame_end(const SamplerArgs& a, const FrameEndArgs& fe, hipStream_t st);
 void launch_ss_to_table(const float* ss, int ss_ld, float* dst, int nss, int rows, hipStream_t st);
 
diff --git a/swift-qwen3-tts_amd/csrc/kernels/sampler.hip b/swift-qwen3-tts_amd/csrc/kernels/sampler.hip
--- a/swift-qwen3-tts_amd/csrc/kernels/sampler.hip
+++ b/swift-qwen3-tts_amd/csrc/kernels/sampler.hip
@@ -6,6 +6,18 @@
 namespace {
 
 constexpr int kMaxVAll = 4096;
+
+#ifdef Q3TTS_SAMPLER_TIMELINE
+__device__ unsigned long long g_sampler_tl[3][64][8];
+#define Q3_STL(k)                                  \
+    do {                                           \
+        __builtin_amdgcn_sched_barrier(0);         \
+        stl_[k] = wall_clock64();                  \
+        __builtin_amdgcn_sched_barrier(0);         \
+    } while (0)
+#else
+#define Q3_STL(k) ((void)0)
+#endif
 
 __device__ __forceinline__ void philox4x32_10(uint32_t c0, uint32_t c1, uint32_t c2, uint32_t c3, uint32_t k0,
                                               uint32_t k1, uint32_t (&out)[4]) {
@@ -133,6 +145,41 @@
     return r;
 }
 
+template <int kThreads>
+__device__ __forceinline__ void next_input(const SamplerArgs& a, int b, int tid, int used, float* red) {
+    if (!a.next_x) return;
+    const int q8 = a.qkv_tab ? a.qkv_ld / 8 : 0;
+    const uint4* qsrc = reinterpret_cast<const uint4*>(a.qkv_tab + (size_t)used * a.qkv_ld);
+    uint4* qdst = reinterpret_cast<uint4*>(a.qkv_out + (size_t)b * a.qkv_ld);
+    uint4 q0 = {0u, 0u, 0u, 0u};
+    if (tid < q8) q0 = qsrc[tid];
+    const uint4* src = reinterpret_cast<const uint4*>(a.emb + (size_t)used * a.emb_ld);
+    float ss = 0.f;
+    for (int i = tid; i < a.H / 8; i += kThreads) {
+        const uint4 v = src[i];
+        const uint32_t w[4] = {v.x, v.y, v.z, v.w};
+#pragma unroll
+        for (int j = 0; j < 4; ++j) ss += lo_bf(w[j]) * lo_bf(w[j]) + hi_bf(w[j]) * hi_bf(w[j]);
+        *reinterpret_cast<uint4*>(a.next_x + act_tiled_offset(b + a.next_row0, 8 * i, a.next_MB)) = v;
+    }
+    if (tid < q8) qdst[tid] = q0;
+    for (int i = tid + kThreads; i < q8; i += kThreads) qdst[i] = qsrc[i];
+    if (a.emb_ss) {
+        for (int j = tid; j < a.nss; j += kThreads)
+            a.next_ss[(size_t)j * a.next_ss_ld + b + a.next_row0] = a.emb_ss[(size_t)used * a.nss + j];
+    } else if (a.next_ss) {
+        ss = wave_sum(ss);
+        __syncthreads();
+        if ((tid & 63) == 0) red[tid >> 6] = ss;
+        __syncthreads();
+        if (tid == 0) {
+            float t = 0.f;
+            for (int w = 0; w < kThreads / 64; ++w) t += red[w];
+            a.next_ss[b] = t;
+        }
+    }
+}
+
 template <int kThreads, int kMaxV, bool TALKER, bool FEND>
 __device__ __forceinline__ void sampler_body(const SamplerArgs& a, const FrameEndArgs* fe) {
     constexpr int kElems = kMaxV / kThreads;
@@ -147,6 +194,10 @@
     __shared__ int sel[2][2];
 
     const int b = blockIdx.x, tid = threadIdx.x;
+#ifdef Q3TTS_SAMPLER_TIMELINE
+    unsigned long long stl_[8] = {0, 0, 0, 0, 0, 0, 0, 0};
+#endif
+    Q3_STL(0);
     const int V = a.V;
     const uint16_t* lrow = a.logits + (size_t)b * a.ldl;
     uint16_t raw[kElems];
@@ -202,6 +253,7 @@
         if (need_vals) vals[k * kThreads + tid] = v;
     }
     __syncthreads();
+    Q3_STL(1);
 
     int tok;
     if (sp.temperature <= 0.f) {
@@ -263,6 +315,8 @@
                 if (level == 0) prefix = (uint32_t)sel[0][0];
                 else prefix = (prefix << 8) | (uint32_t)sel[1][0];
                 need = sel[level][1];
+                if (level == 0) Q3_STL(2);
+                else Q3_STL(3);
             }
             const uint32_t kt = prefix;
             unsigned long long bal[kElems];
@@ -296,6 +350,7 @@
                 for (int k = 0; k < kElems; ++k) vals[k * kThreads + tid] = l[k];
                 __syncthreads();
             }
+            Q3_STL(4);
         }
         if (use_top_p) {
             const int lane = tid & 63;
@@ -362,6 +417,7 @@
             }
         }
         __syncthreads();
+        Q3_STL(5);
         const int ns = n_surv;
         Best x{-INFINITY, 0x7fffffff};
         for (int q = tid; q < ns; q += kThreads) {
@@ -371,6 +427,7 @@
         }
         Best r = block_argmax<kThreads>(x, scratch);
         tok = (r.i == 0x7fffffff) ? 0 : r.i;
+        Q3_STL(6);
     }
 
     int used = tok;
@@ -392,31 +449,14 @@
             if (frame < a.Fmax) a.codes[((size_t)b * a.Fmax + frame) * 16 + a.cb] = used;
         }
     }
-    if (a.next_x) {
-        const uint4* src = reinterpret_cast<const uint4*>(a.emb + (size_t)used * a.emb_ld);
-        float ss = 0.f;
-        for (int i = tid; i < a.H / 8; i += kThreads) {
-            const uint4 v = src[i];
-            const uint32_t w[4] = {v.x, v.y, v.z, v.w};
-#pragma unroll
-            for (int j = 0; j < 4; ++j) ss += lo_bf(w[j]) * lo_bf(w[j]) + hi_bf(w[j]) * hi_bf(w[j]);
-            *reinterpret_cast<uint4*>(a.next_x + act_tiled_offset(b + a.next_row0, 8 * i, a.next_MB)) = v;
-        }
-        if (a.emb_ss) {
-            for (int j = tid; j < a.nss; j += kThreads)
-                a.next_ss[(size_t)j * a.next_ss_ld + b + a.next_row0] = a.emb_ss[(size_t)used * a.nss + j];
-        } else if (a.next_ss) {
-            ss = wave_sum(ss);
-            __syncthreads();
-            if ((tid & 63) == 0) vals[tid >> 6] = ss;
-            __syncthreads();
-            if (tid == 0) {
-                float t = 0.f;
-                for (int w = 0; w < kThreads / 64; ++w) t += vals[w];
-                a.next_ss[b] = t;
-            }
-        }
-    }
+    next_input<kThreads>(a, b, tid, used, vals);
+    Q3_STL(7);
+#ifdef Q3TTS_SAMPLER_TIMELINE
+    if (tid == 0 && b < 64) {
+#pragma unroll
+        for (int k = 0; k < 8; ++k) g_sampler_tl[TALKER ? 1 : (FEND ? 2 : 0)][b][k] = stl_[k];
+    }
+#endif
     if constexpr (FEND) {
         __shared__ float fe_sh[4];
         frame_end_job(*fe, b, tid, used, fe_sh);
@@ -434,6 +474,10 @@
 __global__ __launch_bounds__(1024) void sampler_fend_kernel(SamplerFendArgs a) {
     sampler_body<1024, 2048, false, true>(a.s, &a.fe);
 }
+__global__ __launch_bounds__(1024) void sampler_next_input_kernel(SamplerArgs a, int code0, const int32_t* codes) {
+    __shared__ float red[1024 / 64];
+    next_input<1024>(a, blockIdx.x, threadIdx.x, codes ? codes[blockIdx.x] : code0 + (int)blockIdx.x, red);
+}
 
 }
 
@@ -443,7 +487,13 @@
     hipLaunchKernelGGL(sampler_fend_kernel, dim3(a.B), dim3(1024), 0, st, s);
 }
 
+void launch_sampler_next_input(const SamplerArgs& a, int code0, const int32_t* codes, hipStream_t st) {
+    Q3_CHECK(a.next_x && a.B >= 1 && code0 >= 0 && (!a.qkv_tab || (a.qkv_out && a.qkv_ld % 8 == 0)), 3, "sampler: bad hand-over arguments");
+    hipLaunchKernelGGL(sampler_next_input_kernel, dim3(a.B), dim3(1024), 0, st, a, code0, codes);
+}
+
 void launch_sampler(const SamplerArgs& a, hipStream_t st) {
+    Q3_CHECK(!a.qkv_tab || (a.next_x && a.qkv_out && a.qkv_ld % 8 == 0), 3, "sampler: a q/k/v table needs its output row and next_x");
     Q3_CHECK(a.V <= kMaxVAll, 3, "sampler: vocabulary larger than 4096 is not supported");
     if (!a.is_talker && a.V <= 2048) hipLaunchKernelGGL((sampler_kernel<1024, 2048, false>), dim3(a.B), dim3(1024), 0, st, a);
     else if (a.is_talker) hipLaunchKernelGGL((sampler_kernel<1024, 4096, true>), dim3(a.B), dim3(1024), 0, st, a);
@@ -451,3 +501,10 @@
 }
 
 }
+
+#ifdef Q3TTS_SAMPLER_TIMELINE
+extern "C" int q3tts_debug_sampler_timeline(unsigned long long* out) {
+    if (hipDeviceSynchronize() != hipSuccess) return 7;
+    return hipMemcpyFromSymbol(out, HIP_SYMBOL(q3::g_sampler_tl), sizeof(q3::g_sampler_tl)) == hipSuccess ? 0 : 7;
+}
+#endif
diff --git a/swift-qwen3-tts_amd/csrc/model.h b/swift-qwen3-tts_amd/csrc/model.h
--- a/swift-qwen3-tts_amd/csrc/model.h
+++ b/swift-qwen3-tts_amd/csrc/model.h
@@ -182,6 +182,8 @@
     std::vector<void*> side_allocs;
     mutable std::vector<const uint16_t*> cp_pe;
     mutable std::vector<const float*> cp_pss;
+    mutable const uint16_t* cp_qkv = nullptr;
+    mutable int cp_qkv_ntab = 0;
     mutable std::vector<void*> lazy_allocs;
     mutable std::mutex lazy_mutex;
 
diff --git a/swift-qwen3-tts_amd/qwen3tts/_lib.py b/swift-qwen3-tts_amd/qwen3tts/_lib.py
--- a/swift-qwen3-tts_amd/qwen3tts/_lib.py
+++ b/swift-qwen3-tts_amd/qwen3tts/_lib.py
@@ -299,6 +299,8 @@
                                                  f32p, C.c_int64]
     if hasattr(L, "q3tts_debug_prefix_states"):
         L.q3tts_debug_prefix_states.argtypes = [vp, i32p, C.POINTER(C.c_int64), C.POINTER(C.c_int64)]
+    if hasattr(L, "q3tts_debug_cp_qkv_rows"):
+        L.q3tts_debug_cp_qkv_rows.argtypes = [vp, C.c_int32, i32p, C.c_int32, u16p, u16p, u16p, i32p]
     if hasattr(L, "q3tts_debug_codec_stream_slots"):
         L.q3tts_debug_codec_stream_slots.argtypes = [vp, i32p, i32p, C.c_int32, C.c_int32, C.c_int32, C.c_int32, C.c_int32, C.c_int32,
                                                      C.c_int32, f32p]
diff --git a/swift-qwen3-tts_amd/qwen3tts/model.py b/swift-qwen3-tts_amd/qwen3tts/model.py
--- a/swift-qwen3-tts_amd/qwen3tts/model.py
+++ b/swift-qwen3-tts_amd/qwen3tts/model.py
@@ -647,6 +647,15 @@
                                                                    nf.ctypes.data_as(L.i32p), B, F, int(chunk_frames), int(window),
                                                                    int(lookahead), pcm.ctypes.data_as(L.f32p)))
         return pcm
+
+    def debug_cp_qkv_rows(self, table: int, codes: Sequence[int]):
+        codes = np.ascontiguousarray(codes, np.int32)
+        ld = C.c_int32(0)
+        self._check(self._lib.q3tts_debug_cp_qkv_rows(self._h, table, codes.ctypes.data_as(L.i32p), codes.size, None, None, None, C.byref(ld)))
+        out = [np.zeros((codes.size, ld.value), np.uint16) for _ in range(3)]
+        self._check(self._lib.q3tts_debug_cp_qkv_rows(self._h, table, codes.ctypes.data_as(L.i32p), codes.size,
+                                                      *(o.ctypes.data_as(L.u16p) for o in out), C.byref(ld)))
+        return tuple(out)
 
     def debug_prefix_states(self) -> Tuple[int, int, int]:
         n, b, r = C.c_int32(0), C.c_int64(0), C.c_int64(0)
```

Result: slower. 10380 (-2.2%).
